# facebookresearch/theseus

Measured on NVIDIA H100. Metric: LM iterations/sec on batched SE3 pose-graph (2500 poses, global batch 2048 over N GPUs, LM + block-sparse Cholesky, fp64), higher is better.
Workload: dtype f64

## Files before the change

theseus_b200/_lib.py:

```python
import ctypes as C
import os

_HERE = os.path.dirname(os.path.abspath(__file__))
_LIB_PATH = os.environ.get("THB200_LIB") or os.path.join(_HERE, "lib", "libthb200.so")
_lib = None

c_i32, c_i64, c_f64, c_f32, c_vp = C.c_int32, C.c_int64, C.c_double, C.c_float, C.c_void_p


class CostGroup(C.Structure):
    _fields_ = [("kind", c_i32), ("weight_kind", c_i32), ("K", c_i32), ("dim", c_i32),
                ("x0", c_vp), ("x1", c_vp), ("aux", c_vp), ("w", c_vp), ("bstride", c_vp),
                ("a_off", c_vp), ("a_stride", c_vp), ("bp", c_vp), ("row0", c_vp),
                ("aux2", c_vp), ("aux3", c_vp), ("aux4", c_vp), ("bstride2", c_vp),
                ("robust_kind", c_i32), ("reserved0", c_i32), ("log_radius", c_vp), ("bstride_lr", c_vp),
                ("x2", c_vp), ("x3", c_vp), ("bstride3", c_vp), ("grid_rows", c_i32), ("grid_cols", c_i32)]


class VarTable(C.Structure):
    _fields_ = [("N", c_i32), ("x", c_vp), ("out", c_vp), ("kind", c_vp), ("col", c_vp), ("dof", c_vp)]


class GramPlan(C.Structure):
    _fields_ = [("num_entries", c_i64), ("ent_blk", c_vp), ("ent_p", c_vp), ("ent_q", c_vp),
                ("blk_out", c_vp), ("blk_ld", c_vp), ("blk_mirror", c_vp), ("blk_cptr", c_vp),
                ("c_off", c_vp), ("c_stride", c_vp), ("c_rows", c_vp), ("c_bpa", c_vp), ("c_bpb", c_vp),
                ("n", c_i64), ("col_cptr", c_vp), ("cc_off", c_vp), ("cc_stride", c_vp), ("cc_rows", c_vp),
                ("cc_row0", c_vp), ("num_blocks", c_i64), ("blk_rows", c_vp), ("blk_cols", c_vp),
                ("num_segments", c_i64), ("segments", c_vp), ("blk_order", c_vp)]


def make_gram_plan(arrs, dev):
    return GramPlan(
        num_entries=int(arrs["ent_blk"].shape[0]), ent_blk=dev["ent_blk"].data_ptr(), ent_p=dev["ent_p"].data_ptr(),
        ent_q=dev["ent_q"].data_ptr(), blk_out=dev["blk_out"].data_ptr(), blk_ld=dev["blk_ld"].data_ptr(),
        blk_mirror=dev["blk_mirror"].data_ptr(), blk_cptr=dev["blk_cptr"].data_ptr(), c_off=dev["c_off"].data_ptr(),
        c_stride=dev["c_stride"].data_ptr(), c_rows=dev["c_rows"].data_ptr(), c_bpa=dev["c_bpa"].data_ptr(),
        c_bpb=dev["c_bpb"].data_ptr(), n=int(arrs["n"]), col_cptr=dev["col_cptr"].data_ptr(),
        cc_off=dev["cc_off"].data_ptr(), cc_stride=dev["cc_stride"].data_ptr(), cc_rows=dev["cc_rows"].data_ptr(),
        cc_row0=dev["cc_row0"].data_ptr(), num_blocks=int(arrs["blk_out"].shape[0]), blk_rows=dev["blk_rows"].data_ptr(),
        blk_cols=dev["blk_cols"].data_ptr(), num_segments=int(arrs["segments"].shape[0]), segments=arrs["segments"].ctypes.data,
        blk_order=dev["blk_order"].data_ptr())


class SparsePlanStruct(C.Structure):
    _fields_ = [("N", c_i32), ("num_levels", c_i32), ("max_dim", c_i32), ("reserved", c_i32),
                ("n", c_i64), ("data_size", c_i64), ("winv_size", c_i64)] + [(k, c_vp) for k in (
                    "dims", "col_start", "pstart", "winv_off", "diag_off", "up_a", "up_b", "up_k",
                    "u_ptr", "u_tgt", "u_r", "u_c", "u_ld", "u_p0", "u_p1",
                    "f_ptr", "f_off", "f_dim", "f_w", "f_col",
                    "t_ptr", "t_off", "t_r", "t_dim", "t_w",
                    "s_ptr", "s_col", "fr_ptr", "fr_off", "fr_k", "bc_ptr", "bc_off", "bc_i")]


class SparseLanePlanStruct(C.Structure):
    _fields_ = [("N", c_i64), ("n", c_i64), ("data_size", c_i64), ("diag_size", c_i64), ("num_launches", c_i64)] + [(k, c_vp) for k in (
        "launches", "dims", "col_start", "pstart", "dl_off", "diag_off", "up_a", "up_b", "up_k", "u_tgt", "u_p0", "u_p1",
        "t_off", "t_diag", "t_dl", "t_pstart", "s_col", "fr_ptr", "fr_off", "fr_p", "fr_d", "bc_ptr", "bc_off", "bc_p", "bc_d")]


_PG, _PV, _PP = C.POINTER(CostGroup), C.POINTER(VarTable), C.POINTER(GramPlan)
_PS = C.POINTER(SparsePlanStruct)
_PL = C.POINTER(SparseLanePlanStruct)


class SparseLaneRootStruct(C.Structure):
    _fields_ = [("num_blocks", c_i64), ("num_cols", c_i64), ("nt", c_i64), ("root_start", c_i64), ("num_segments", c_i64)] + [(k, c_vp) for k in (
        "segments", "rb_off", "rb_row", "rb_col", "rb_di", "rb_dj", "rf_p0", "rf_p1", "root_cols", "root_dims")]


class SparseLaneTilesStruct(C.Structure):
    _fields_ = [("num_tiles", c_i64), ("num_steps", c_i64), ("tile_tgt", c_vp), ("step_ptr", c_vp), ("step_src", c_vp)]


class SparseLanePiecesStruct(C.Structure):
    _fields_ = [("num_pieces", c_i64), ("num_launches", c_i64)] + [(k, c_vp) for k in (
        "launches", "first", "width", "fr_ext_end", "bc_int_end", "order")]


class FrontPlanStruct(C.Structure):
    _fields_ = [("S", c_i64), ("n", c_i64), ("data_size", c_i64), ("arena_size", c_i64), ("varena_size", c_i64)] + [(k, c_vp) for k in (
        "f_w", "f_b", "f_first", "f_class", "f_wpad", "f_np", "f_cb_ld", "f_depth", "f_panel_off", "f_cb_off", "f_fr_off", "f_u_off",
        "child_ptr", "child_list", "rel_ptr", "f_rel", "rows_ptr", "f_rows", "sched", "perm", "c_jw", "c_sp_ptr", "c_sp", "c_inv_ptr", "c_inv", "fd", "pc", "pmap")]


_PF = C.POINTER(FrontPlanStruct)
_PR = C.POINTER(SparseLaneRootStruct)
_PPIECES = C.POINTER(SparseLanePiecesStruct)
_PT = C.POINTER(SparseLaneTilesStruct)
SIGNATURES = {
    "thb_version": (c_i32, []),
    "thb_compiled_arch": (c_i32, []),
    "thb_launch_count": (c_i64, []),
    "thb_linearize_group_f64": (c_i32, [_PG, c_i64, c_vp, c_i64, c_vp, c_i64, c_vp]),
    "thb_linearize_group_f32": (c_i32, [_PG, c_i64, c_vp, c_i64, c_vp, c_i64, c_vp]),
    "thb_error_num_chunks": (c_i32, [c_i32]),
    "thb_error_group_f64": (c_i32, [_PG, c_i64, c_vp, c_vp]),
    "thb_error_group_f32": (c_i32, [_PG, c_i64, c_vp, c_vp]),
    "thb_error_reduce_f64": (c_i32, [c_vp, c_i32, c_i64, c_vp, c_vp]),
    "thb_error_reduce_f32": (c_i32, [c_vp, c_i32, c_i64, c_vp, c_vp]),
    "thb_retract_f64": (c_i32, [_PV, c_i64, c_vp, c_i64, c_f64, c_vp, c_vp]),
    "thb_retract_f32": (c_i32, [_PV, c_i64, c_vp, c_i64, c_f32, c_vp, c_vp]),
    "thb_commit_f64": (c_i32, [_PV, c_i64, c_vp, c_vp]),
    "thb_commit_f32": (c_i32, [_PV, c_i64, c_vp, c_vp]),
    "thb_gram_f64": (c_i32, [_PP, c_i64, c_vp, c_i64, c_vp, c_i64, c_vp, c_i64, c_vp, c_vp, c_vp]),
    "thb_gram_f32": (c_i32, [_PP, c_i64, c_vp, c_i64, c_vp, c_i64, c_vp, c_i64, c_vp, c_vp, c_vp]),
    "thb_fill_zero": (c_i32, [c_vp, c_i64, c_vp]),
    "thb_potrf_workspace_bytes": (c_i64, [c_i64, c_i64]),
    "thb_potrf_f64": (c_i32, [c_vp, c_vp, c_vp, c_vp, c_i64, c_i64, c_vp, c_i64, c_vp]),
    "thb_potrs_f64": (c_i32, [c_vp, c_vp, c_i64, c_i64, c_vp, c_i64, c_vp]),
    "thb_potrf_potrs_f64": (c_i32, [c_vp, c_vp, c_vp, c_vp, c_vp, c_vp, c_i64, c_i64, c_vp, c_i64, c_vp]),
    "thb_sparse_damp_f64": (c_i32, [_PS, c_vp, c_vp, c_vp, c_i64, c_vp]),
    "thb_sparse_factor_f64": (c_i32, [_PS, c_vp, c_vp, c_vp, c_i64, c_vp]),
    "thb_sparse_solve_f64": (c_i32, [_PS, c_vp, c_vp, c_vp, c_vp, c_vp, c_i64, c_vp]),
    "thb_symbolic_create": (c_i32, [c_vp, c_i64, c_vp, c_vp, c_i32, c_vp]),
    "thb_symbolic_destroy": (None, [c_vp]),
    "thb_symbolic_array_count": (c_i64, [c_vp, C.c_char_p]),
    "thb_symbolic_array_elem_bytes": (c_i32, [c_vp, C.c_char_p]),
    "thb_symbolic_array_copy": (c_i32, [c_vp, C.c_char_p, c_vp, c_i64]),
    "thb_symbolic_stat": (C.c_double, [c_vp, C.c_char_p]),
    "thb_sparse_lane_padded_batch": (c_i64, [c_i64]),
    "thb_sparse_lane_gram_f64": (c_i32, [_PP, c_i64, c_vp, c_i64, c_vp, c_vp]),
    "thb_sparse_lane_damp_f64": (c_i32, [_PL, c_vp, c_vp, c_vp, c_i64, c_vp]),
    "thb_sparse_lane_factor_f64": (c_i32, [_PL, c_vp, c_vp, c_vp, c_i64, c_vp]),
    "thb_sparse_lane_factor_tiled_f64": (c_i32, [_PL, _PT, c_vp, c_vp, c_vp, c_i64, c_vp]),
    "thb_sparse_lane_solve_f64": (c_i32, [_PL, c_vp, c_vp, c_vp, c_vp, c_vp, c_i64, c_vp]),
    "thb_sparse_lane_forward_f64": (c_i32, [_PL, c_vp, c_vp, c_vp, c_vp, c_i64, c_vp]),
    "thb_sparse_lane_backward_f64": (c_i32, [_PL, c_vp, c_vp, c_vp, c_vp, c_i64, c_vp]),
    "thb_sparse_lane_piece_forward_f64": (c_i32, [_PL, _PPIECES, c_vp, c_vp, c_vp, c_vp, c_i64, c_vp]),
    "thb_sparse_lane_piece_backward_f64": (c_i32, [_PL, _PPIECES, c_vp, c_vp, c_vp, c_vp, c_i64, c_vp]),
    "thb_sparse_lane_root_gather_f64": (c_i32, [_PR, c_vp, c_vp, c_i64, c_vp]),
    "thb_sparse_lane_root_rhs_f64": (c_i32, [_PL, _PR, c_vp, c_vp, c_vp, c_vp, c_i64, c_vp]),
    "thb_sparse_lane_root_scatter_f64": (c_i32, [_PL, _PR, c_vp, c_vp, c_vp, c_i64, c_vp]),
    "thb_gram_dense_f64": (c_i32, [c_vp, c_vp, c_i64, c_i64, c_i64, c_vp]),
    "thb_front_small_smem_bytes": (c_i64, [c_i32, c_i32, c_i32]),
    "thb_front_factor_f64": (c_i32, [_PF, c_vp, c_i64, c_vp, c_vp, c_i64, c_vp, c_vp, c_vp, c_vp, c_i64, c_vp, c_i64, c_vp]),
    "thb_front_solve_f64": (c_i32, [_PF, c_vp, c_i64, c_vp, c_vp, c_vp, c_vp, c_vp, c_i64, c_vp]),
    "thb_front_factor_forward_f64": (c_i32, [_PF, c_vp, c_i64, c_vp, c_vp, c_i64, c_vp, c_vp, c_vp, c_vp, c_i64, c_vp, c_vp, c_vp, c_vp,
                                             c_i64, c_vp]),
    "thb_front_forward_f64": (c_i32, [_PF, c_vp, c_i64, c_vp, c_vp, c_vp, c_vp, c_i64, c_vp]),
    "thb_front_backward_f64": (c_i32, [_PF, c_vp, c_i64, c_vp, c_vp, c_vp, c_i64, c_vp]),
    "thb_potrf_partial_workspace_bytes": (c_i64, [c_i64, c_i64]),
    "thb_potrf_partial_inplace_f64": (c_i32, [c_vp, c_i64, c_i64, c_i32, c_i32, c_i32, c_i32, c_vp, c_i64, c_vp, c_i64, c_vp]),
    "thb_solve_backward_f64": (c_i32, [c_i64, c_i64, c_i64, c_vp, c_vp, c_vp, c_vp, c_vp, c_vp, c_vp, c_i32, c_vp, c_vp, c_vp]),
    "thb_lm_control_f64": (c_i32, [c_vp, c_vp, c_vp, c_i64, c_i64, c_f64, c_vp, c_vp, c_vp, c_i32, c_f64, c_f64, c_f64,
                                   c_vp, c_vp, c_vp, c_vp]),
    "thb_lm_control_f32": (c_i32, [c_vp, c_vp, c_vp, c_i64, c_i64, c_f32, c_vp, c_vp, c_vp, c_i32, c_f32, c_f32, c_f32,
                                   c_vp, c_vp, c_vp, c_vp]),
    "thb_mat_vec_f64": (c_i32, [c_i64, c_i64, c_i64, c_vp, c_vp, c_vp, c_vp, c_vp, c_vp]),
    "thb_tmat_vec_f64": (c_i32, [c_i64, c_i64, c_i64, c_vp, c_vp, c_vp, c_vp, c_vp, c_vp]),
}
for _sfx, _ in (("f64", c_f64), ("f32", c_f32)):
    SIGNATURES[f"thb_se3_exp_{_sfx}"] = (c_i32, [c_vp, c_vp, c_i64, c_vp])
    SIGNATURES[f"thb_se3_log_{_sfx}"] = (c_i32, [c_vp, c_vp, c_vp, c_i64, c_vp])
    SIGNATURES[f"thb_se3_adjoint_{_sfx}"] = (c_i32, [c_vp, c_vp, c_i64, c_vp])
    SIGNATURES[f"thb_se3_inverse_{_sfx}"] = (c_i32, [c_vp, c_vp, c_i64, c_vp])
    SIGNATURES[f"thb_se3_compose_{_sfx}"] = (c_i32, [c_vp, c_vp, c_vp, c_i64, c_vp])
    SIGNATURES[f"thb_se3_jexp_{_sfx}"] = (c_i32, [c_vp, c_vp, c_vp, c_i64, c_vp])
    SIGNATURES[f"thb_so3_jexp_{_sfx}"] = (c_i32, [c_vp, c_vp, c_vp, c_i64, c_vp])
    for _g in ("so3", "se2"):
        SIGNATURES[f"thb_{_g}_exp_{_sfx}"] = (c_i32, [c_vp, c_vp, c_i64, c_vp])
        SIGNATURES[f"thb_{_g}_log_{_sfx}"] = (c_i32, [c_vp, c_vp, c_vp, c_i64, c_vp])
        SIGNATURES[f"thb_{_g}_adjoint_{_sfx}"] = (c_i32, [c_vp, c_vp, c_i64, c_vp])
        SIGNATURES[f"thb_{_g}_inverse_{_sfx}"] = (c_i32, [c_vp, c_vp, c_i64, c_vp])
        SIGNATURES[f"thb_{_g}_compose_{_sfx}"] = (c_i32, [c_vp, c_vp, c_vp, c_i64, c_vp])


def lib_path():
    return _LIB_PATH


def load():
    global _lib
    if _lib is not None:
        return _lib
    if not os.path.exists(_LIB_PATH):
        raise RuntimeError(
            f"libthb200.so not found at {_LIB_PATH}: build it with `python -m theseus_b200.build` "
            "(theseus_b200 has no CPU or PyTorch fallback for its compute path)")
    import torch
    lib = C.CDLL(_LIB_PATH, mode=C.RTLD_GLOBAL)
    for name, (res, args) in SIGNATURES.items():
        fn = getattr(lib, name)
        fn.restype = res
        fn.argtypes = args
    _lib = lib
    return lib


replayed_launches = 0


def total_launches() -> int:
    return int(load().thb_launch_count()) + replayed_launches


def check(rc, what):
    if rc != 0:
        kind = "invalid argument" if rc < 0 else "CUDA error"
        raise RuntimeError(f"libthb200: {what} failed with {kind} code {rc}")


def stream_ptr():
    import torch
    return C.c_void_p(torch.cuda.current_stream().cuda_stream)


def ptr(t):
    return None if t is None else C.c_void_p(t.data_ptr())
```

theseus_b200/csrc/thb_front.cu:

```cuda
#include <stdlib.h>

#include "thb_common.cuh"

namespace thb {

#ifdef THB_SIMT_EMU
#define THB_PDL_TRIGGER() do { } while (0)
#define THB_PDL_WAIT() do { } while (0)
#define FRONT_LAUNCH(K, grid, block, smem, cs, arg) K<<<grid, block, smem, cs>>>(arg)
#else
#define THB_PDL_TRIGGER() asm volatile("griddepcontrol.launch_dependents;" ::: "memory")
#define THB_PDL_WAIT() asm volatile("griddepcontrol.wait;" ::: "memory")
#define FRONT_LAUNCH(K, grid, block, smem, cs, arg) thb::front_launch_pdl(K, grid, block, smem, cs, arg)
static inline bool front_pdl_enabled() {
  static const bool on = [] { const char* e = getenv("THB_FRONT_PDL"); return e != nullptr && e[0] == '1'; }();
  return on;
}
template <typename A>
static inline void front_launch_pdl(void (*kernel)(A), dim3 grid, dim3 block, size_t smem, cudaStream_t cs, const A& arg) {
  cudaLaunchConfig_t cfg = {};
  cfg.gridDim = grid; cfg.blockDim = block; cfg.dynamicSmemBytes = smem; cfg.stream = cs;
  cudaLaunchAttribute at[1];
  at[0].id = cudaLaunchAttributeProgrammaticStreamSerialization;
  at[0].val.programmaticStreamSerializationAllowed = 1;
  cfg.attrs = at; cfg.numAttrs = front_pdl_enabled() ? 1 : 0;
  cudaLaunchKernelEx(&cfg, kernel, arg);
}
#endif

#ifdef THB_SIMT_EMU
__device__ inline void front_mma884(double& c0, double& c1, double a, double b) {
  const int lane = threadIdx.x & 31, lr = lane >> 2, lc = lane & 3;
  for (int k = 0; k < 4; k++) {
    const double av = __shfl_sync(0xffffffffu, a, lr * 4 + k);
    const double b0 = __shfl_sync(0xffffffffu, b, (2 * lc) * 4 + k);
    const double b1 = __shfl_sync(0xffffffffu, b, (2 * lc + 1) * 4 + k);
    c0 += av * b0;
    c1 += av * b1;
  }
}
#else
__device__ __forceinline__ void front_mma884(double& c0, double& c1, double a, double b) {
  asm volatile("mma.sync.aligned.m8n8k4.row.col.f64.f64.f64.f64 {%0,%1}, {%2}, {%3}, {%0,%1};\n" : "+d"(c0), "+d"(c1) : "d"(a), "d"(b));
}
#endif

__host__ __device__ __forceinline__ int front_pad_ld(int x) { return ((x + 11) / 16) * 16 + 4; }

struct FrontArgs {
  thb_front_plan p;
  int s0;
  int64_t B;
  double* factor;
  const double* alpha;
  const double* beta;
  double* arena_cur;
  const double* arena_child;
  int32_t* info;
  int prefetch;
  const double* ata;
  int64_t ata_stride;
  const double* rhs;
  double* work;
  double* v_cur;
  const double* v_child;
};

__device__ __forceinline__ double front_panel_in(const FrontArgs& a, const double* Lg, int64_t poff, int64_t item, int64_t e) {
  if (a.ata == nullptr) return Lg[e];
  const int32_t m = a.p.pmap[poff + e];
  return m >= 0 ? a.ata[item * a.ata_stride + m] : 0.0;
}

constexpr int FRONT_WD_LD = 20;
#ifndef FRONT_PL
#define FRONT_PL 4
#endif
constexpr int FRONT_MAX_CHILDREN = 8;

__host__ __device__ __forceinline__ int64_t front_smem_doubles(int w, int b, int nchildren) {
  const int b16 = (b + 15) & ~15, w8 = (w + 7) & ~7;
  return (int64_t)(w8 + b16 + 8) * front_pad_ld(w8) + 8 * FRONT_WD_LD + 3 * FRONT_MAX_CHILDREN
         + ((int64_t)nchildren * (w + b) + 1) / 2 + 2;
}

__device__ __forceinline__ int front_leaf8(double* __restrict__ T, int ld, double* __restrict__ Wd, int lane) {
  const int ln = lane < 8 ? lane : 0;
  double row[8];
#pragma unroll
  for (int q = 0; q < 8; q++) row[q] = T[ln * ld + q];
  int fail = 0;
  double invd = 0.0;
#pragma unroll
  for (int c = 0; c < 8; c++) {
    const double d = __shfl_sync(0xffffffffu, row[c], c);
    if (!(d > 0.0) && fail == 0) fail = c + 1;
    double inv = rsqrt(d);
    inv = inv * (1.5 - 0.5 * d * inv * inv);
    const double sq = d * inv;
    if (lane == c) invd = inv;
    const double lrc = (lane == c) ? sq : row[c] * inv;
    row[c] = lrc;
#pragma unroll
    for (int q = c + 1; q < 8; q++) {
      const double lqc = __shfl_sync(0xffffffffu, lrc, q);
      row[q] -= lrc * lqc;
    }
  }
  if (lane < 8) {
#pragma unroll
    for (int q = 0; q < 8; q++)
      if (q <= lane) T[lane * ld + q] = row[q];
  }
  double x[8];
#pragma unroll
  for (int rr = 0; rr < 8; rr++) {
    double sacc = (lane == rr) ? 1.0 : 0.0;
#pragma unroll
    for (int k = 0; k < rr; k++) {
      const double lrk = __shfl_sync(0xffffffffu, row[k], rr);
      sacc -= lrk * x[k];
    }
    x[rr] = sacc * __shfl_sync(0xffffffffu, invd, rr);
  }
  if (lane < 8) {
#pragma unroll
    for (int rr = 0; rr < 8; rr++) Wd[rr * FRONT_WD_LD + lane] = (rr >= lane) ? x[rr] : 0.0;
  }
  return fail;
}

__device__ __forceinline__ void front_diag_block(double* PN, int ldp, int jb, double* Wd, int lane, int w, int first, int32_t* info) {
  const int lr = lane >> 2, lc = lane & 3;
  double c0 = 0.0, c1 = 0.0;
  const double* Arow = PN + (8 * jb + lr) * ldp + lc;
  for (int k = 0; k < 8 * jb; k += 4) {
    const double av = Arow[k];
    front_mma884(c0, c1, av, av);
  }
  double* d = PN + (8 * jb + lr) * ldp + 8 * jb + 2 * lc;
  d[0] -= c0;
  d[1] -= c1;
  __syncwarp();
  const int fail = front_leaf8(PN + (8 * jb) * ldp + 8 * jb, ldp, Wd, lane);
  if (lane == 0 && fail != 0 && 8 * jb + fail <= w) atomicCAS(info, 0, first + 8 * jb + fail);
}

template <bool TWO>
__device__ __forceinline__ void front_tile_column(double* PN, int ldp, int jb, int rt0, const double* Wd, int lane) {
  const int lr = lane >> 2, lc = lane & 3;
  double x00 = 0.0, x01 = 0.0, x10 = 0.0, x11 = 0.0;
  const double* A0 = PN + (8 * rt0 + lr) * ldp + lc;
  const double* Bj = PN + (8 * jb + lr) * ldp + lc;
  for (int k = 0; k < 8 * jb; k += 4) {
    const double bf = Bj[k];
    front_mma884(x00, x01, A0[k], bf);
    if (TWO) front_mma884(x10, x11, A0[8 * ldp + k], bf);
  }
  double* X0 = PN + (8 * rt0 + lr) * ldp + 8 * jb + 2 * lc;
  X0[0] -= x00; X0[1] -= x01;
  if (TWO) { X0[8 * ldp] -= x10; X0[8 * ldp + 1] -= x11; }
  __syncwarp();
  x00 = x01 = x10 = x11 = 0.0;
#pragma unroll
  for (int k = 0; k < 8; k += 4) {
    const double bf = Wd[lr * FRONT_WD_LD + k + lc];
    front_mma884(x00, x01, A0[8 * jb + k], bf);
    if (TWO) front_mma884(x10, x11, A0[8 * ldp + 8 * jb + k], bf);
  }
  __syncwarp();
  X0[0] = x00; X0[1] = x01;
  if (TWO) { X0[8 * ldp] = x10; X0[8 * ldp + 1] = x11; }
}

struct FrontChild {
  const double* src;
  int ldg, lo, hi, uoff;
};

__device__ __forceinline__ double front_warp_trsv_lower(const double* T, int ld, double ui, int cw, int lane) {
  const double rd = lane < cw ? 1.0 / T[lane * ld + lane] : 0.0;
  for (int k = 0; k < cw; k++) {
    const double yk = __shfl_sync(0xffffffffu, ui * rd, k);
    if (lane == k) ui = yk;
    else if (lane > k && lane < cw) ui -= T[lane * ld + k] * yk;
  }
  return ui;
}

struct FrontRowsGlobal {
  static constexpr bool kInPanel = false;
  const double* L;
  int w;
  double* T;
  __device__ __forceinline__ const double* row(int i) const { return L + (int64_t)i * w; }
  __device__ __forceinline__ const double* diag(int k0, int cw, int tid, int nthreads, int* ld) const {
    for (int e = tid; e < cw * cw; e += nthreads) {
      const int i = e / cw, j = e - i * cw;
      T[i * 33 + j] = L[(int64_t)(k0 + i) * w + k0 + j];
    }
    *ld = 33;
    return T;
  }
};
struct FrontRowsPanel {
  static constexpr bool kInPanel = true;
  const double* PN;
  int ldp, w, shift;
  __device__ __forceinline__ const double* row(int i) const { return PN + (i < w ? i : i + shift) * ldp; }
  __device__ __forceinline__ const double* diag(int k0, int, int, int, int* ld) const {
    *ld = ldp;
    return PN + k0 * ldp + k0;
  }
};

template <int THREADS, typename Rows>
__device__ __forceinline__ void front_forward_elim(const Rows& R, double* u, int us, int w, int r, int tid, int lane) {
  for (int k0 = 0; k0 < w; k0 += 32) {
    const int cw = min(32, w - k0);
    int ld;
    const double* T = R.diag(k0, cw, tid, THREADS, &ld);
    __syncthreads();
    if (tid < 32) {
      const double ui = front_warp_trsv_lower(T, ld, lane < cw ? u[(k0 + lane) * us] : 0.0, cw, lane);
      if (lane < cw) u[(k0 + lane) * us] = ui;
    }
    __syncthreads();
    for (int i = k0 + cw + tid; i < r; i += THREADS) {
      const double* row = R.row(i) + k0;
      double s = 0.0;
      if constexpr (Rows::kInPanel) {
#pragma unroll 2
        for (int k = 0; k < cw; k++) s += row[k] * u[(k0 + k) * us];
      } else {
        for (int k = 0; k < cw; k++) s += row[k] * u[(k0 + k) * us];
      }
      u[i * us] -= s;
    }
    __syncthreads();
  }
}

template <int THREADS>
__global__ void __launch_bounds__(THREADS, 1024 / THREADS) front_small_kernel(FrontArgs a) {
  extern __shared__ double sm[];
  const thb_front_plan& p = a.p;
  const int tid = threadIdx.x, lane = tid & 31, warp = tid >> 5;
  constexpr int NW = THREADS / 32;
  const int lr = lane >> 2, lc = lane & 3;
  const int64_t item = blockIdx.x;
  THB_PDL_TRIGGER();
  const int64_t* FD = p.fd + (int64_t)(a.s0 + blockIdx.y) * 8;
  const int t = (int)FD[0];
  const int w = (int)FD[1], b = (int)FD[2], r = w + b;
  const int f_first = (int)FD[3];
  const int64_t f_panel_off = FD[4], f_cb_off = FD[5];
  const int f_cb_ld = (int)FD[6];
  const int c_begin = (int)(FD[7] & 0xffffffffLL);
  const int nch = min((int)(FD[7] >> 32), FRONT_MAX_CHILDREN);
  const int b16 = (b + 15) & ~15, w8 = (w + 7) & ~7;
  const int ldp = front_pad_ld(w8);
  const int prow = w8 + b16 + 8;
  double* PN = sm;
  double* Wd = PN + prow * ldp;
  FrontChild* ch = reinterpret_cast<FrontChild*>(Wd + 8 * FRONT_WD_LD);
  int32_t* INV = reinterpret_cast<int32_t*>(Wd + 8 * FRONT_WD_LD + 3 * FRONT_MAX_CHILDREN);
  for (int q = 0; q < nch; q++) {
    const int64_t* PC = p.pc + (int64_t)(c_begin + q) * 6;
    const double* csrc = a.arena_child + item * p.arena_size + PC[0];
    const int cld = (int)(PC[1] & 0xffffffffLL), cbc = (int)(PC[1] >> 32);
    if (tid == 0) {
      ch[q].src = csrc;
      ch[q].ldg = cld;
      ch[q].lo = (int)PC[2];
      ch[q].hi = (int)PC[3];
      ch[q].uoff = (int)PC[5];
    }
    const int32_t* inv = p.c_inv + PC[4];
    for (int l = tid; l < r; l += THREADS) INV[q * r + l] = inv[l];
    (void)cbc;
  }
  for (int e = tid; e < prow * ldp; e += THREADS) sm[e] = 0.0;
  THB_PDL_WAIT();
#ifndef THB_SIMT_EMU
  if (a.rhs != nullptr) {
    for (int i = tid; i < w; i += THREADS) asm volatile("prefetch.global.L2 [%0];\n" ::"l"(a.rhs + item * p.n + p.perm[f_first + i]));
    for (int q = 0; q < nch; q++) {
      const int64_t* PC = p.pc + (int64_t)(c_begin + q) * 6;
      const double* cu = a.v_child + item * p.varena_size + PC[5];
      for (int off = tid * 16; off < (int)(PC[1] >> 32); off += THREADS * 16) asm volatile("prefetch.global.L2 [%0];\n" ::"l"(cu + off));
    }
  }
  for (int q = 0; a.prefetch != 0 && q < nch; q++) {
    const int64_t* PC = p.pc + (int64_t)(c_begin + q) * 6;
    const double* csrc = a.arena_child + item * p.arena_size + PC[0];
    const int cld = (int)(PC[1] & 0xffffffffLL), cbc = (int)(PC[1] >> 32);
    for (int off = tid * 16; off < cbc * cld; off += THREADS * 16) {
      const int i = off / cld, j = off - i * cld;
      if (j <= i) asm volatile("prefetch.global.L2 [%0];\n" ::"l"(csrc + off));
    }
  }
#endif
  __syncthreads();
  if (tid < w8 - w) PN[(w + tid) * ldp + w + tid] = 1.0;
  double* Lg = a.factor + item * p.data_size + f_panel_off;
  {
    const double al = a.alpha != nullptr ? a.alpha[item] : 0.0;
    const double be = a.beta != nullptr ? a.beta[item] : 0.0;
    const int total = r * w;
    for (int e0 = tid; e0 < total; e0 += FRONT_PL * THREADS) {
      int ii[FRONT_PL], jj[FRONT_PL];
      double v[FRONT_PL];
#pragma unroll
      for (int u = 0; u < FRONT_PL; u++) {
        const int e = e0 + u * THREADS;
        ii[u] = e / w;
        jj[u] = e - ii[u] * w;
        if (e >= total || jj[u] > ii[u]) ii[u] = -1;
        v[u] = ii[u] >= 0 ? front_panel_in(a, Lg, f_panel_off, item, e) : 0.0;
      }
#pragma unroll
      for (int u = 0; u < FRONT_PL; u++)
        if (ii[u] >= 0 && ii[u] == jj[u]) v[u] = v[u] + (al * v[u] + be);
      for (int q = 0; q < nch; q++) {
        const double* src = ch[q].src;
        const int ldg = ch[q].ldg, lo = ch[q].lo, hi = ch[q].hi;
        const int32_t* inv = INV + q * r;
#pragma unroll
        for (int u = 0; u < FRONT_PL; u++) {
          if (ii[u] >= lo && jj[u] <= hi) {
            const int ci = inv[ii[u]], cj = inv[jj[u]];
            if (ci >= 0 && cj >= 0) v[u] += src[(int64_t)ci * ldg + cj];
          }
        }
      }
#pragma unroll
      for (int u = 0; u < FRONT_PL; u++)
        if (ii[u] >= 0) PN[(ii[u] < w ? ii[u] : ii[u] + (w8 - w)) * ldp + jj[u]] = v[u];
    }
  }
  double* U = PN + w8;
  if (a.rhs != nullptr) {
    for (int i = tid; i < r; i += THREADS) {
      double v = i < w ? a.rhs[item * p.n + p.perm[f_first + i]] : 0.0;
      for (int q = 0; q < nch; q++) {
        if (i >= ch[q].lo && i <= ch[q].hi) {
          const int k = INV[q * r + i];
          if (k >= 0) v += a.v_child[item * p.varena_size + ch[q].uoff + k];
        }
      }
      U[i * ldp] = v;
    }
  }
  __syncthreads();
  const int nbk = w8 / 8, nrt = (w8 + b16) / 8;
  for (int jb = 0; jb < nbk; jb++) {
    if (warp == 0) front_diag_block(PN, ldp, jb, Wd, lane, w, f_first, a.info + item);
    __syncthreads();
    const int npair = (nrt - jb) / 2;
    for (int q = warp; q < npair; q += NW) front_tile_column<true>(PN, ldp, jb, jb + 1 + 2 * q, Wd, lane);
    __syncthreads();
  }
  {
    int i = tid / w, j = tid - i * w;
    const int di = THREADS / w, dj = THREADS - di * w;
    for (int e = tid; e < r * w; e += THREADS) {
      Lg[e] = (j > i) ? 0.0 : PN[(i < w ? i : i + (w8 - w)) * ldp + j];
      i += di; j += dj;
      if (j >= w) { j -= w; i++; }
    }
  }
  if (a.rhs != nullptr) {
    front_forward_elim<THREADS>(FrontRowsPanel{PN, ldp, w, w8 - w}, U, ldp, w, r, tid, lane);
    for (int i = tid; i < w; i += THREADS) a.work[item * p.n + f_first + i] = U[i * ldp];
    double* ub = a.v_cur + item * p.varena_size + p.f_u_off[t];
    for (int i = tid; i < b; i += THREADS) ub[i] = U[(w + i) * ldp];
  }
  if (b == 0) return;
  double* dst = a.arena_cur + item * p.arena_size + f_cb_off;
  const int ldg_out = f_cb_ld;
  const double* P = PN + w8 * ldp;
  const int nmt = b16 / 16, ntl = nmt * (nmt + 1) / 2;
  for (int q = warp; q < ntl; q += NW) {
    int R = (int)((sqrtf(8.0f * (float)q + 1.0f) - 1.0f) * 0.5f);
    while ((R + 1) * (R + 2) / 2 <= q) R++;
    while (R * (R + 1) / 2 > q) R--;
    const int ct = q - R * (R + 1) / 2;
    double gch[2][2][2] = {{{0.0, 0.0}, {0.0, 0.0}}, {{0.0, 0.0}, {0.0, 0.0}}};
    const int li0 = w + 16 * R + lr, lj0 = w + 16 * ct + 2 * lc;
    for (int qc = 0; qc < nch; qc++) {
      if (w + 16 * R + 15 >= ch[qc].lo && w + 16 * ct <= ch[qc].hi) {
        const int32_t* inv = INV + qc * r;
        const double* src = ch[qc].src;
        const int ldg = ch[qc].ldg;
        int ci[2], cj[2][2];
#pragma unroll
        for (int mi = 0; mi < 2; mi++) ci[mi] = (li0 + 8 * mi < r) ? inv[li0 + 8 * mi] : -1;
#pragma unroll
        for (int ni = 0; ni < 2; ni++)
#pragma unroll
          for (int u = 0; u < 2; u++) cj[ni][u] = (lj0 + 8 * ni + u < r) ? inv[lj0 + 8 * ni + u] : -1;
#pragma unroll
        for (int mi = 0; mi < 2; mi++)
#pragma unroll
          for (int ni = 0; ni < 2; ni++)
#pragma unroll
            for (int u = 0; u < 2; u++)
              if (ci[mi] >= 0 && cj[ni][u] >= 0 && cj[ni][u] <= ci[mi]) gch[mi][ni][u] += src[(int64_t)ci[mi] * ldg + cj[ni][u]];
      }
    }
    double acc[2][2][2] = {{{0.0, 0.0}, {0.0, 0.0}}, {{0.0, 0.0}, {0.0, 0.0}}};
    const double* Pa = P + (16 * R + lr) * ldp + lc;
    const double* Pb = P + (16 * ct + lr) * ldp + lc;
    for (int k4 = 0; k4 < w8; k4 += 4) {
      const double a0 = Pa[k4], a1 = Pa[8 * ldp + k4];
      const double b0 = Pb[k4], b1 = Pb[8 * ldp + k4];
      front_mma884(acc[0][0][0], acc[0][0][1], a0, b0);
      front_mma884(acc[0][1][0], acc[0][1][1], a0, b1);
      front_mma884(acc[1][0][0], acc[1][0][1], a1, b0);
      front_mma884(acc[1][1][0], acc[1][1][1], a1, b1);
    }
#pragma unroll
    for (int mi = 0; mi < 2; mi++)
#pragma unroll
      for (int ni = 0; ni < 2; ni++) {
        acc[mi][ni][0] = gch[mi][ni][0] - acc[mi][ni][0];
        acc[mi][ni][1] = gch[mi][ni][1] - acc[mi][ni][1];
      }
#pragma unroll
    for (int mi = 0; mi < 2; mi++) {
      const int i = 16 * R + 8 * mi + lr;
      if (i < b) {
        double* drow = dst + (int64_t)i * ldg_out;
#pragma unroll
        for (int ni = 0; ni < 2; ni++)
#pragma unroll
          for (int u = 0; u < 2; u++) {
            const int jj = 16 * ct + 8 * ni + 2 * lc + u;
            if (jj <= i) drow[jj] = acc[mi][ni][u];
          }
      }
    }
  }
}

constexpr int ASM_ROWS = 16, ASM_THREADS = 256;

__device__ __forceinline__ int front_map_big(int l, int w, int wpad) { return l < w ? l : wpad + (l - w); }

__global__ void __launch_bounds__(ASM_THREADS) front_assemble_kernel(FrontArgs a, int t) {
  extern __shared__ double sm[];
  const thb_front_plan& p = a.p;
  const int tid = threadIdx.x;
  const int64_t item = blockIdx.x;
  const int w = p.f_w[t], b = p.f_b[t], r = w + b, wpad = p.f_wpad[t], np = p.f_np[t];
  const int R0 = blockIdx.y * ASM_ROWS;
  const int nc = min(np, 128 * (R0 / 128 + 1));
  const int c_first = p.child_ptr[t], n_children = p.child_ptr[t + 1] - c_first;
  if (n_children <= FRONT_MAX_CHILDREN) {
    const double* Lgg = a.factor + item * p.data_size + p.f_panel_off[t];
    const double alg = a.alpha != nullptr ? a.alpha[item] : 0.0;
    const double beg = a.beta != nullptr ? a.beta[item] : 0.0;
    double* Fg = a.arena_cur + item * p.arena_size + p.f_fr_off[t] + (int64_t)R0 * np;
    __shared__ const double* s_src[FRONT_MAX_CHILDREN];
    __shared__ const int32_t* s_inv[FRONT_MAX_CHILDREN];
    __shared__ int s_ld[FRONT_MAX_CHILDREN];
    if (tid < n_children) {
      const int c = p.child_list[c_first + tid];
      s_src[tid] = a.arena_child + item * p.arena_size + p.f_cb_off[c];
      s_inv[tid] = p.c_inv + p.c_inv_ptr[c];
      s_ld[tid] = p.f_cb_ld[c];
    }
    __syncthreads();
    const int64_t poff = p.f_panel_off[t];
    const int total = ASM_ROWS * nc;
    for (int e0 = tid; e0 < total; e0 += 4 * ASM_THREADS) {
      int li[4], lj[4];
      double v[4];
#pragma unroll
      for (int u = 0; u < 4; u++) {
        const int e = e0 + u * ASM_THREADS;
        const int rr = e / nc, fc = e - rr * nc;
        const int fr = R0 + rr;
        li[u] = fr < w ? fr : ((fr >= wpad && fr - wpad + w < r) ? fr - wpad + w : -1);
        lj[u] = fc < w ? fc : ((fc >= wpad && fc - wpad + w < r) ? fc - wpad + w : -1);
        v[u] = 0.0;
        if (e >= total) {
          li[u] = lj[u] = -2;
        } else if (li[u] < 0 || lj[u] < 0) {
          v[u] = (fr == fc) ? 1.0 : 0.0;
          li[u] = -1;
        } else if (lj[u] > li[u]) {
          li[u] = -1;
        } else if (lj[u] < w) {
          v[u] = front_panel_in(a, Lgg, poff, item, (int64_t)li[u] * w + lj[u]);
        }
      }
#pragma unroll
      for (int u = 0; u < 4; u++)
        if (li[u] >= 0 && li[u] == lj[u] && lj[u] < w) v[u] = v[u] + (alg * v[u] + beg);
      for (int q = 0; q < n_children; q++) {
        const double* src = s_src[q];
        const int32_t* inv = s_inv[q];
        const int ldg = s_ld[q];
        int ci[4], cj[4];
#pragma unroll
        for (int u = 0; u < 4; u++) {
          ci[u] = li[u] >= 0 ? inv[li[u]] : -1;
          cj[u] = li[u] >= 0 ? inv[lj[u]] : -1;
        }
#pragma unroll
        for (int u = 0; u < 4; u++)
          if (ci[u] >= 0 && cj[u] >= 0) v[u] += src[(int64_t)ci[u] * ldg + cj[u]];
      }
#pragma unroll
      for (int u = 0; u < 4; u++) {
        const int e = e0 + u * ASM_THREADS;
        if (e < total) Fg[e + (int64_t)(e / nc) * (np - nc)] = v[u];
      }
    }
    return;
  }
  double* buf = sm;
  for (int e = tid; e < ASM_ROWS * nc; e += ASM_THREADS) buf[e] = 0.0;
  __syncthreads();
  const double* Lg = a.factor + item * p.data_size + p.f_panel_off[t];
  const double al = a.alpha != nullptr ? a.alpha[item] : 0.0;
  const double be = a.beta != nullptr ? a.beta[item] : 0.0;
  const int wlim = min(wpad, nc);
  for (int e = tid; e < ASM_ROWS * wlim; e += ASM_THREADS) {
    const int rr = e / wlim, j = e - rr * wlim;
    const int fr = R0 + rr;
    int i = -1;
    if (fr < w) i = fr;
    else if (fr >= wpad && fr - wpad + w < r) i = fr - wpad + w;
    if (i >= 0) {
      if (j < w && !(i < w && j > i)) {
        double v = front_panel_in(a, Lg, p.f_panel_off[t], item, (int64_t)i * w + j);
        if (i == j) v = v + (al * v + be);
        buf[rr * nc + j] = v;
      }
    } else if (j == fr) {
      buf[rr * nc + j] = 1.0;
    }
  }
  for (int rr = tid; rr < ASM_ROWS; rr += ASM_THREADS) {
    const int fr = R0 + rr;
    if (fr >= wpad + b) buf[rr * nc + fr] = 1.0;
  }
  __syncthreads();
  for (int ci = p.child_ptr[t]; ci < p.child_ptr[t + 1]; ci++) {
    const int c = p.child_list[ci];
    const int bc = p.f_b[c], ldg = p.f_cb_ld[c];
    const int32_t* rel = p.f_rel + p.rel_ptr[c];
    int lo = 0, hi = bc;
    while (lo < hi) { const int mid = (lo + hi) >> 1; if (front_map_big(rel[mid], w, wpad) < R0) lo = mid + 1; else hi = mid; }
    const int i0 = lo;
    hi = bc;
    while (lo < hi) { const int mid = (lo + hi) >> 1; if (front_map_big(rel[mid], w, wpad) < R0 + ASM_ROWS) lo = mid + 1; else hi = mid; }
    const int i1 = lo;
    if (i1 > i0) {
      const double* src = a.arena_child + item * p.arena_size + p.f_cb_off[c];
      for (int i = i0 + (tid >> 5); i < i1; i += ASM_THREADS / 32) {
        const int fr = front_map_big(rel[i], w, wpad) - R0;
        const double* srow = src + (int64_t)i * ldg;
        for (int j = tid & 31; j <= i; j += 32) buf[fr * nc + front_map_big(rel[j], w, wpad)] += srow[j];
      }
      __syncthreads();
    }
  }
  double* F = a.arena_cur + item * p.arena_size + p.f_fr_off[t] + (int64_t)R0 * np;
  for (int e = tid; e < ASM_ROWS * nc; e += ASM_THREADS) {
    const int rr = e / nc, c = e - rr * nc;
    F[(int64_t)rr * np + c] = buf[e];
  }
}

__global__ void __launch_bounds__(256) front_extract_kernel(FrontArgs a, int t) {
  const thb_front_plan& p = a.p;
  const int64_t item = blockIdx.x;
  const int w = p.f_w[t], b = p.f_b[t], r = w + b, wpad = p.f_wpad[t], np = p.f_np[t];
  const double* F = a.arena_cur + item * p.arena_size + p.f_fr_off[t];
  double* Lg = a.factor + item * p.data_size + p.f_panel_off[t];
  for (int e = blockIdx.y * blockDim.x + threadIdx.x; e < r * w; e += gridDim.y * blockDim.x) {
    const int i = e / w, j = e - i * w;
    const int fr = i < w ? i : wpad + (i - w);
    Lg[e] = (i < w && j > i) ? 0.0 : F[(int64_t)fr * np + j];
  }
}

struct FrontSolveArgs {
  thb_front_plan p;
  int s0;
  int64_t B;
  const double* factor;
  const double* rhs;
  double* x;
  double* work;
  double* v_cur;
  const double* v_child;
  int stage_doubles;
};

__device__ __forceinline__ double front_warp_trsv_upper(const double* T, double ti, int cw, int lane) {
  const double rd = lane < cw ? 1.0 / T[lane * 33 + lane] : 0.0;
  for (int k = cw - 1; k >= 0; k--) {
    const double xk = __shfl_sync(0xffffffffu, ti * rd, k);
    if (lane == k) ti = xk;
    else if (lane < k) ti -= T[k * 33 + lane] * xk;
  }
  return ti;
}

template <int THREADS>
__global__ void __launch_bounds__(THREADS) front_forward_kernel(FrontSolveArgs a) {
  extern __shared__ double sm[];
  const thb_front_plan& p = a.p;
  const int tid = threadIdx.x, lane = tid & 31;
  const int64_t item = blockIdx.x;
  THB_PDL_TRIGGER();
  const int64_t* FD = p.fd + (int64_t)(a.s0 + blockIdx.y) * 8;
  const int t = (int)FD[0];
  const int w = (int)FD[1], b = (int)FD[2], r = w + b, first = (int)FD[3];
  THB_PDL_WAIT();
  double* u = sm;
  double* T = sm + ((r + 1) & ~1);
  const double* Lg = a.factor + item * p.data_size + FD[4];
  if (r * w <= a.stage_doubles) {
    double* Ls = T + 32 * 33 + 1 + (THREADS & ~1) + 2;
    for (int e = tid; e < r * w; e += THREADS) Ls[e] = Lg[e];
    Lg = Ls;
  }
  {
    const int c0 = (int)(FD[7] & 0xffffffffLL), nchild = (int)(FD[7] >> 32);
    for (int i = tid; i < r; i += THREADS) {
      double v = i < w ? a.rhs[item * p.n + p.perm[first + i]] : 0.0;
      for (int q = 0; q < nchild; q++) {
        const int64_t* PC = p.pc + (int64_t)(c0 + q) * 6;
        if (i >= (int)PC[2] && i <= (int)PC[3]) {
          const int k = p.c_inv[PC[4] + i];
          if (k >= 0) v += a.v_child[item * p.varena_size + PC[5] + k];
        }
      }
      u[i] = v;
    }
  }
  __syncthreads();
  front_forward_elim<THREADS>(FrontRowsGlobal{Lg, w, T}, u, 1, w, r, tid, lane);
  for (int i = tid; i < w; i += THREADS) a.work[item * p.n + first + i] = u[i];
  if (b > 0) {
    double* ub = a.v_cur + item * p.varena_size + p.f_u_off[t];
    for (int i = tid; i < b; i += THREADS) ub[i] = u[w + i];
  }
}

template <int THREADS>
__global__ void __launch_bounds__(THREADS) front_backward_kernel(FrontSolveArgs a) {
  extern __shared__ double sm[];
  const thb_front_plan& p = a.p;
  const int tid = threadIdx.x, lane = tid & 31, warp = tid >> 5;
  const int64_t item = blockIdx.x;
  THB_PDL_TRIGGER();
  const int64_t* FD = p.fd + (int64_t)(a.s0 + blockIdx.y) * 8;
  const int t = (int)FD[0];
  const int w = (int)FD[1], b = (int)FD[2], r = w + b, first = (int)FD[3];
  THB_PDL_WAIT();
  double* xf = sm;
  double* T = sm + ((r + 1) & ~1);
  double* part = T + 32 * 33 + 1;
  const double* Lg = a.factor + item * p.data_size + FD[4];
  if (r * w <= a.stage_doubles) {
    double* Ls = T + 32 * 33 + 1 + (THREADS & ~1) + 2;
    for (int e = tid; e < r * w; e += THREADS) Ls[e] = Lg[e];
    Lg = Ls;
  }
  double* wk = a.work + item * p.n;
  const int32_t* rows = p.f_rows + p.rows_ptr[t];
  for (int i = tid; i < r; i += THREADS) xf[i] = i < w ? wk[first + i] : wk[rows[i - w]];
  __syncthreads();
  const int nchunk = (w + 31) / 32;
  for (int ch = nchunk - 1; ch >= 0; ch--) {
    const int k0 = ch * 32, cw = min(32, w - k0);
    const int RG = THREADS / cw;
    const int kk = tid % cw, rg = tid / cw;
    for (int e = tid; e < cw * cw; e += THREADS) {
      const int i = e / cw, j = e - i * cw;
      T[i * 33 + j] = Lg[(int64_t)(k0 + i) * w + k0 + j];
    }
    double acc = 0.0;
    if (rg < RG) {
      const double* col = Lg + k0 + kk;
      int i = k0 + cw + rg;
      for (; i + 3 * RG < r; i += 4 * RG) {
        const double l0 = col[(int64_t)i * w], l1 = col[(int64_t)(i + RG) * w], l2 = col[(int64_t)(i + 2 * RG) * w],
                     l3 = col[(int64_t)(i + 3 * RG) * w];
        acc += l0 * xf[i];
        acc += l1 * xf[i + RG];
        acc += l2 * xf[i + 2 * RG];
        acc += l3 * xf[i + 3 * RG];
      }
      for (; i < r; i += RG) acc += col[(int64_t)i * w] * xf[i];
    }
    part[tid] = acc;
    __syncthreads();
    if (warp == 0) {
      double tk = 0.0;
      if (lane < cw) {
        tk = xf[k0 + lane];
        for (int g = 0; g < RG; g++) tk -= part[g * cw + lane];
      }
      tk = front_warp_trsv_upper(T, tk, cw, lane);
      if (lane < cw) xf[k0 + lane] = tk;
    }
    __syncthreads();
  }
  for (int i = tid; i < w; i += THREADS) {
    const double v = xf[i];
    wk[first + i] = v;
    a.x[item * p.n + p.perm[first + i]] = v;
  }
}

static inline int front_threads_of_class(int cls) { return cls == 0 ? 64 : (cls == 1 ? 128 : 256); }

template <typename K>
static inline int front_set_smem(K kernel, size_t bytes, size_t* cache) {
  if (bytes > *cache) {
    cudaError_t e = cudaFuncSetAttribute(kernel, cudaFuncAttributeMaxDynamicSharedMemorySize, (int)bytes);
    if (e != cudaSuccess) return (int)e;
    *cache = bytes;
  }
  return 0;
}

static int front_solve_launch(const thb_front_plan* p, const int64_t* L, int pass, const double* factor, const double* rhs, double* x,
                              double* work, double* varena, int64_t B, cudaStream_t cs) {
  static size_t fw_set[3] = {0, 0, 0}, bw_set[3] = {0, 0, 0};
  static const int64_t stage_cap = [] { const char* e = getenv("THB_SOLVE_STAGE"); return e != nullptr ? (int64_t)atoll(e) : (int64_t)0; }();
  const int depth = (int)L[0], cls = (int)L[1], begin = (int)L[2], count = (int)L[3];
  FrontSolveArgs a;
  a.p = *p; a.s0 = begin; a.B = B; a.factor = factor; a.rhs = rhs; a.x = x; a.work = work;
  a.v_cur = varena != nullptr ? varena + (int64_t)(depth & 1) * B * p->varena_size : nullptr;
  a.v_child = varena != nullptr ? varena + (int64_t)((depth + 1) & 1) * B * p->varena_size : nullptr;
  const int kc = cls > 2 ? 2 : cls;
  const int threads = front_threads_of_class(kc);
  const int64_t r_max = L[5];
  const int64_t stage = (cls < 3 && L[6] > 0) ? (L[6] < stage_cap ? L[6] : stage_cap) : 0;
  a.stage_doubles = (int)stage;
  const size_t smem = (size_t)(((r_max + 1) & ~1LL) + 32 * 33 + 1 + threads + 2 + stage + 2) * 8;
  const dim3 grid((unsigned)B, (unsigned)count);
  if (pass == 0) {
    if (kc == 0) { int rc = front_set_smem(front_forward_kernel<64>, smem, &fw_set[0]); if (rc) return rc;
                   FRONT_LAUNCH(front_forward_kernel<64>, grid, 64, smem, cs, a); }
    else if (kc == 1) { int rc = front_set_smem(front_forward_kernel<128>, smem, &fw_set[1]); if (rc) return rc;
                        FRONT_LAUNCH(front_forward_kernel<128>, grid, 128, smem, cs, a); }
    else { int rc = front_set_smem(front_forward_kernel<256>, smem, &fw_set[2]); if (rc) return rc;
           FRONT_LAUNCH(front_forward_kernel<256>, grid, 256, smem, cs, a); }
  } else {
    if (kc == 0) { int rc = front_set_smem(front_backward_kernel<64>, smem, &bw_set[0]); if (rc) return rc;
                   FRONT_LAUNCH(front_backward_kernel<64>, grid, 64, smem, cs, a); }
    else if (kc == 1) { int rc = front_set_smem(front_backward_kernel<128>, smem, &bw_set[1]); if (rc) return rc;
                        FRONT_LAUNCH(front_backward_kernel<128>, grid, 128, smem, cs, a); }
    else { int rc = front_set_smem(front_backward_kernel<256>, smem, &bw_set[2]); if (rc) return rc;
           FRONT_LAUNCH(front_backward_kernel<256>, grid, 256, smem, cs, a); }
  }
  THB_CHECK_LAUNCH();
  return THB_OK;
}

static int front_factor(const thb_front_plan* p, const int64_t* launches, int64_t num_launches, double* factor, const double* ata,
                        int64_t ata_stride, const double* alpha, const double* beta, double* arena, void* dense_ws, int64_t dense_ws_bytes,
                        int32_t* info, const double* rhs, double* work, double* varena, int64_t B, thb_stream_t stream) {
  if (p == nullptr || launches == nullptr || factor == nullptr || arena == nullptr || info == nullptr || B < 0) return THB_ERR_BAD_ARG;
  if (B == 0 || p->S == 0) return THB_OK;
  if (B > 65535LL * 32768LL) return THB_ERR_UNSUPPORTED;
  cudaStream_t cs = thb_cs(stream);
  THB_CUDA(cudaMemsetAsync(info, 0, (size_t)B * 4, cs));
  static size_t smem_set[5] = {0, 0, 0, 0, 0}, asm_set = 0;
  static const int thr_cls[2] = {[] { const char* e = getenv("THB_FRONT_T0"); const int v = e ? atoi(e) : 64; return (v == 128 || v == 256) ? v : 64; }(),
                                 [] { const char* e = getenv("THB_FRONT_T1"); const int v = e ? atoi(e) : 128; return v == 256 ? 256 : 128; }()};
  static int front_prefetch_flag = -1;
  if (front_prefetch_flag < 0) {
    const char* e = getenv("THB_FRONT_PREFETCH");
    front_prefetch_flag = (e != nullptr && e[0] == '1') ? 1 : 0;
  }
  static const int fuse_max = [] { const char* e = getenv("THB_FRONT_FUSE_MAX"); return e != nullptr ? atoi(e) : 1024; }();
  for (int64_t l = 0; l < num_launches; l++) {
    const int64_t* L = launches + l * THB_FRONT_LAUNCH_COLS;
    const int depth = (int)L[0], cls = (int)L[1], begin = (int)L[2], count = (int)L[3];
    FrontArgs a;
    a.p = *p; a.s0 = begin; a.B = B; a.factor = factor; a.alpha = alpha; a.beta = beta; a.info = info;
    a.ata = (ata != nullptr && p->pmap != nullptr) ? ata : nullptr; a.ata_stride = ata_stride;
    a.prefetch = front_prefetch_flag;
    a.arena_cur = arena + (int64_t)(depth & 1) * B * p->arena_size;
    a.arena_child = arena + (int64_t)((depth + 1) & 1) * B * p->arena_size;
    a.rhs = rhs; a.work = work;
    a.v_cur = rhs != nullptr ? varena + (int64_t)(depth & 1) * B * p->varena_size : nullptr;
    a.v_child = rhs != nullptr ? varena + (int64_t)((depth + 1) & 1) * B * p->varena_size : nullptr;
    if (cls < 3) {
      const size_t smem = (size_t)L[4];
#ifndef THB_SIMT_EMU
      if (smem > 227 * 1024) return THB_ERR_UNSUPPORTED;
#endif
      const dim3 grid((unsigned)B, (unsigned)count);
      if (count > 65535) return THB_ERR_UNSUPPORTED;
      const int threads = (cls == 0 && thr_cls[0] == 64) ? 64
                          : ((cls == 0 && thr_cls[0] == 128) || (cls == 1 && thr_cls[1] == 128)) ? 128
                          : (cls <= 1 || smem <= 56 * 1024) ? 256 : (smem <= 113 * 1024 ? 512 : 1024);
      const bool fused = rhs != nullptr && threads <= fuse_max;
      if (!fused) a.rhs = nullptr;
      if (threads == 64) {
        int rc = front_set_smem(front_small_kernel<64>, smem, &smem_set[0]); if (rc) return rc;
        FRONT_LAUNCH(front_small_kernel<64>, grid, 64, smem, cs, a);
      } else if (threads == 128) {
        int rc = front_set_smem(front_small_kernel<128>, smem, &smem_set[1]); if (rc) return rc;
        FRONT_LAUNCH(front_small_kernel<128>, grid, 128, smem, cs, a);
      } else if (threads == 256) {
        int rc = front_set_smem(front_small_kernel<256>, smem, &smem_set[2]); if (rc) return rc;
        FRONT_LAUNCH(front_small_kernel<256>, grid, 256, smem, cs, a);
      } else if (threads == 512) {
        int rc = front_set_smem(front_small_kernel<512>, smem, &smem_set[3]); if (rc) return rc;
        FRONT_LAUNCH(front_small_kernel<512>, grid, 512, smem, cs, a);
      } else {
        int rc = front_set_smem(front_small_kernel<1024>, smem, &smem_set[4]); if (rc) return rc;
        FRONT_LAUNCH(front_small_kernel<1024>, grid, 1024, smem, cs, a);
      }
      THB_CHECK_LAUNCH();
      if (rhs != nullptr && !fused) {
        const int rc = front_solve_launch(p, L, 0, factor, rhs, nullptr, work, varena, B, cs);
        if (rc != THB_OK) return rc;
      }
    } else {
      const int64_t np = L[5], nb_piv = L[6], fr_off = L[7], first = L[8];
      const int t = (int)L[9];
#ifdef THB_SIMT_EMU
      (void)np; (void)nb_piv; (void)fr_off; (void)first; (void)t; (void)dense_ws; (void)dense_ws_bytes; (void)asm_set;
      return THB_ERR_UNSUPPORTED;
#else
      if (dense_ws == nullptr || np % 128 != 0 || np > 8192) return THB_ERR_BAD_ARG;
      const size_t smem = (size_t)ASM_ROWS * np * 8;
      int rc = front_set_smem(front_assemble_kernel, smem, &asm_set); if (rc) return rc;
      front_assemble_kernel<<<dim3((unsigned)B, (unsigned)(np / ASM_ROWS)), ASM_THREADS, smem, cs>>>(a, t);
      THB_CHECK_LAUNCH();
      rc = thb_potrf_partial_inplace_f64(a.arena_cur + fr_off, p->arena_size, np, (int32_t)nb_piv, (int32_t)L[10], (int32_t)(nb_piv * 64 + L[11]),
                                         (int32_t)first, info, B, dense_ws, dense_ws_bytes, stream);
      if (rc != THB_OK) return rc;
      front_extract_kernel<<<dim3((unsigned)B, 8), 256, 0, cs>>>(a, t);
      THB_CHECK_LAUNCH();
      if (rhs != nullptr) {
        rc = front_solve_launch(p, L, 0, factor, rhs, nullptr, work, varena, B, cs);
        if (rc != THB_OK) return rc;
      }
#endif
    }
  }
  return THB_OK;
}

}

extern "C" {

int64_t thb_front_small_smem_bytes(int32_t w, int32_t b, int32_t nchildren) { return thb::front_smem_doubles(w, b, nchildren) * 8; }

int thb_front_factor_f64(const thb_front_plan* p, const int64_t* launches, int64_t num_launches, double* factor, const double* ata,
                         int64_t ata_stride, const double* alpha, const double* beta, double* arena, void* dense_ws, int64_t dense_ws_bytes,
                         int32_t* info, int64_t B, thb_stream_t stream) {
  return thb::front_factor(p, launches, num_launches, factor, ata, ata_stride, alpha, beta, arena, dense_ws, dense_ws_bytes, info, nullptr,
                           nullptr, nullptr, B, stream);
}

int thb_front_factor_forward_f64(const thb_front_plan* p, const int64_t* launches, int64_t num_launches, double* factor, const double* ata,
                                 int64_t ata_stride, const double* alpha, const double* beta, double* arena, void* dense_ws,
                                 int64_t dense_ws_bytes, int32_t* info, const double* rhs, double* work, double* varena, int64_t B,
                                 thb_stream_t stream) {
  if (rhs == nullptr || work == nullptr || varena == nullptr) return THB_ERR_BAD_ARG;
  return thb::front_factor(p, launches, num_launches, factor, ata, ata_stride, alpha, beta, arena, dense_ws, dense_ws_bytes, info, rhs, work,
                           varena, B, stream);
}

int thb_front_solve_f64(const thb_front_plan* p, const int64_t* launches, int64_t num_launches, const double* factor, const double* rhs,
                        double* x, double* work, double* varena, int64_t B, thb_stream_t stream) {
  if (p == nullptr || launches == nullptr || factor == nullptr || rhs == nullptr || x == nullptr || work == nullptr || varena == nullptr ||
      B < 0)
    return THB_ERR_BAD_ARG;
  if (B == 0 || p->S == 0) return THB_OK;
  const int rc = thb_front_forward_f64(p, launches, num_launches, factor, rhs, work, varena, B, stream);
  if (rc != THB_OK) return rc;
  return thb_front_backward_f64(p, launches, num_launches, factor, x, work, B, stream);
}

int thb_front_forward_f64(const thb_front_plan* p, const int64_t* launches, int64_t num_launches, const double* factor, const double* rhs,
                          double* work, double* varena, int64_t B, thb_stream_t stream) {
  if (p == nullptr || launches == nullptr || factor == nullptr || rhs == nullptr || work == nullptr || varena == nullptr || B < 0)
    return THB_ERR_BAD_ARG;
  if (B == 0 || p->S == 0) return THB_OK;
  cudaStream_t cs = thb_cs(stream);
  for (int64_t q = 0; q < num_launches; q++) {
    const int rc = thb::front_solve_launch(p, launches + q * THB_FRONT_LAUNCH_COLS, 0, factor, rhs, nullptr, work, varena, B, cs);
    if (rc != THB_OK) return rc;
  }
  return THB_OK;
}

int thb_front_backward_f64(const thb_front_plan* p, const int64_t* launches, int64_t num_launches, const double* factor, double* x,
                           double* work, int64_t B, thb_stream_t stream) {
  if (p == nullptr || launches == nullptr || factor == nullptr || x == nullptr || work == nullptr || B < 0) return THB_ERR_BAD_ARG;
  if (B == 0 || p->S == 0) return THB_OK;
  cudaStream_t cs = thb_cs(stream);
  for (int64_t q = num_launches - 1; q >= 0; q--) {
    const int rc = thb::front_solve_launch(p, launches + q * THB_FRONT_LAUNCH_COLS, 1, factor, nullptr, x, work, nullptr, B, cs);
    if (rc != THB_OK) return rc;
  }
  return THB_OK;
}

}
```

theseus_b200/extlib.py:

```python
import ctypes as C
from typing import Dict, Tuple

import numpy as np
import torch

from . import _lib
from .frontal import FrontPlan, build_front_plan


class SymbolicDecomposition:
    def __init__(self, param_size: torch.Tensor, sparse_struct_ptrs: torch.Tensor, sparse_struct_inds: torch.Tensor, dev: str = "cuda"):
        if str(dev) not in ("cuda",) and not str(dev).startswith("cuda"):
            raise RuntimeError("theseus_b200.extlib: only dev='cuda' exists (no CPU implementation of the factorisation in this package)")
        ps = np.asarray(param_size.cpu().numpy() if torch.is_tensor(param_size) else param_size, dtype=np.int64)
        ptrs = np.asarray(sparse_struct_ptrs.cpu().numpy() if torch.is_tensor(sparse_struct_ptrs) else sparse_struct_ptrs, dtype=np.int64)
        inds = np.asarray(sparse_struct_inds.cpu().numpy() if torch.is_tensor(sparse_struct_inds) else sparse_struct_inds, dtype=np.int64)
        N = int(ps.shape[0])
        if ptrs.shape[0] != N + 1:
            raise RuntimeError("sparse_struct_ptrs must have len(param_size) + 1 entries")
        nbr = [set([i]) for i in range(N)]
        for i in range(N):
            for j in inds[ptrs[i]:ptrs[i + 1]]:
                nbr[i].add(int(j)); nbr[int(j)].add(i)
        fp = np.zeros(N + 1, dtype=np.int64)
        fi = []
        for i in range(N):
            fi.extend(sorted(nbr[i])); fp[i + 1] = len(fi)
        self.param_size = ps
        self.plan: FrontPlan = build_front_plan(ps, fp, np.array(fi, dtype=np.int64))
        self.device = torch.device(dev if str(dev) != "cuda" else "cuda")
        self.param_start = np.concatenate([[0], np.cumsum(ps)[:-1]]).astype(np.int64)
        self.to_param = np.repeat(np.arange(N), ps)
        self._dev = None
        self._tables: Dict[Tuple, Tuple[torch.Tensor, ...]] = {}

    def create_numeric_decomposition(self, batch_size: int) -> "NumericDecomposition":
        return NumericDecomposition(self, int(batch_size))

    def _device_plan(self):
        if self._dev is None:
            P = self.plan
            dev = {k: torch.from_numpy(np.ascontiguousarray(v)).to(self.device) for k, v in P.arrays.items()}
            keys = ("f_w", "f_b", "f_first", "f_class", "f_wpad", "f_np", "f_cb_ld", "f_depth", "f_panel_off", "f_cb_off", "f_fr_off", "f_u_off",
                    "child_ptr", "child_list", "rel_ptr", "f_rel", "rows_ptr", "f_rows", "sched", "perm", "c_jw", "c_sp_ptr", "c_sp", "c_inv_ptr", "c_inv", "fd", "pc", "pmap")
            st = _lib.FrontPlanStruct(S=P.S, n=P.n, data_size=P.data_size, arena_size=P.arena_size, varena_size=P.varena_size,
                                      **{k: dev[k].data_ptr() for k in keys})
            launches = np.ascontiguousarray(P.launches, dtype=np.int64)
            big = launches[launches[:, 1] == 3]
            self._dev = dict(front=st, keep=dev, launches=launches, max_np=int(big[:, 5].max()) if len(big) else 0)
        return self._dev

    def _offset_of(self, r: np.ndarray, c: np.ndarray) -> np.ndarray:
        P = self.plan
        A = P.arrays
        pr, pc = self.to_param[r], self.to_param[c]
        posr, posc = P.pos[pr], P.pos[pc]
        swap = posr < posc
        r2, c2 = np.where(swap, c, r), np.where(swap, r, c)
        pr, pc = self.to_param[r2], self.to_param[c2]
        posr, posc = P.pos[pr], P.pos[pc]
        same = posr == posc
        sw2 = same & (r2 < c2)
        r2, c2 = np.where(sw2, c2, r2), np.where(sw2, r2, c2)
        gr = P.pstart[posr] + (r2 - self.param_start[pr])
        gc = P.pstart[posc] + (c2 - self.param_start[pc])
        s = P.front_of_pos[posc]
        first, w = A["f_first"][s].astype(np.int64), A["f_w"][s].astype(np.int64)
        lcol = gc - first
        out = np.empty(r.shape[0], dtype=np.int64)
        for k in range(r.shape[0]):
            if gr[k] < first[k] + w[k]:
                lrow = gr[k] - first[k]
                if lrow < lcol[k]:
                    lrow, lc = lcol[k], gr[k] - first[k]
                    out[k] = A["f_panel_off"][s[k]] + lrow * w[k] + lc
                    continue
            else:
                rows = P.border_rows[int(s[k])]
                j = int(np.searchsorted(rows, gr[k]))
                assert rows[j] == gr[k], "entry outside the symbolic structure"
                lrow = w[k] + j
            out[k] = A["f_panel_off"][s[k]] + lrow * w[k] + lcol[k]
        return out

    def _add_m_table(self, ptrs: np.ndarray, inds: np.ndarray):
        key = ("M", ptrs.tobytes(), inds.tobytes())
        if key not in self._tables:
            rows = np.repeat(np.arange(ptrs.shape[0] - 1), np.diff(ptrs))
            keep = np.nonzero(inds <= rows)[0]
            off = self._offset_of(rows[keep], inds[keep])
            self._tables[key] = (torch.from_numpy(keep).to(self.device), torch.from_numpy(off).to(self.device))
        return self._tables[key]

    def _add_mtm_table(self, ptrs: np.ndarray, inds: np.ndarray):
        key = ("MtM", ptrs.tobytes(), inds.tobytes())
        if key not in self._tables:
            jj, ii = [], []
            for q in range(ptrs.shape[0] - 1):
                a, b = int(ptrs[q]), int(ptrs[q + 1])
                for j in range(a, b):
                    for i in range(a, j + 1):
                        jj.append(j); ii.append(i)
            jj, ii = np.array(jj, dtype=np.int64), np.array(ii, dtype=np.int64)
            off = self._offset_of(inds[jj], inds[ii])
            order = np.argsort(off, kind="stable")
            self._tables[key] = tuple(torch.from_numpy(x[order]).to(self.device) for x in (jj, ii, off))
        return self._tables[key]

    def _diag_offsets(self):
        if "diag" not in self._tables:
            idx = np.arange(self.plan.n)
            self._tables["diag"] = (torch.from_numpy(self._offset_of(idx, idx)).to(self.device),)
        return self._tables["diag"][0]


class NumericDecomposition:
    def __init__(self, symbolic: SymbolicDecomposition, batch_size: int):
        self.sym, self.B = symbolic, batch_size
        P = symbolic.plan
        self.data = torch.zeros(batch_size, P.data_size, dtype=torch.float64, device=symbolic.device)
        self._bufs = None

    @staticmethod
    def _np(t):
        return np.ascontiguousarray(t.cpu().numpy() if torch.is_tensor(t) else t, dtype=np.int64)

    def add_M(self, val: torch.Tensor, ptrs, inds):
        keep, off = self.sym._add_m_table(self._np(ptrs), self._np(inds))
        self.data.index_add_(1, off, val.to(self.data.device, torch.float64)[:, keep])

    def add_MtM(self, val: torch.Tensor, ptrs, inds):
        jj, ii, off = self.sym._add_mtm_table(self._np(ptrs), self._np(inds))
        v = val.to(self.data.device, torch.float64)
        self.data.index_add_(1, off, v[:, jj] * v[:, ii])

    def damp(self, alpha: torch.Tensor, beta: torch.Tensor):
        d = self.sym._diag_offsets()
        diag = self.data[:, d]
        self.data[:, d] = diag * (1.0 + alpha.to(diag).view(-1, 1)) + beta.to(diag).view(-1, 1)

    def _buffers(self):
        if self._bufs is None:
            P, dev = self.sym.plan, self.sym._device_plan()
            lib = _lib.load()
            ws_bytes = int(lib.thb_potrf_partial_workspace_bytes(self.B, dev["max_np"])) if dev["max_np"] else 0
            kw = dict(dtype=torch.float64, device=self.data.device)
            self._bufs = dict(arena=torch.empty(2, self.B, P.arena_size, **kw), varena=torch.empty(2, self.B, P.varena_size, **kw),
                              work=torch.empty(self.B, P.n, **kw), ws=torch.empty(max(ws_bytes, 8), dtype=torch.uint8, device=self.data.device),
                              info=torch.empty(self.B, dtype=torch.int32, device=self.data.device))
        return self._bufs

    def factor(self):
        dev, bufs, lib = self.sym._device_plan(), self._buffers(), _lib.load()
        L = dev["launches"]
        _lib.check(lib.thb_front_factor_f64(C.byref(dev["front"]), L.ctypes.data, L.shape[0], _lib.ptr(self.data), None, 0, None, None, _lib.ptr(bufs["arena"]),
                                            _lib.ptr(bufs["ws"]) if dev["max_np"] else None, bufs["ws"].numel(), _lib.ptr(bufs["info"]), self.B,
                                            _lib.stream_ptr()), "front_factor")
        bad = bufs["info"].nonzero()
        if bad.numel() > 0:
            k = int(bad[0, 0])
            raise RuntimeError(f"block-sparse Cholesky: batch element {k}: matrix is not positive definite (pivot {int(bufs['info'][k])})")

    def solve(self, x: torch.Tensor):
        dev, bufs, lib = self.sym._device_plan(), self._buffers(), _lib.load()
        L = dev["launches"]
        rhs = x.detach().to(torch.float64).contiguous().clone()
        out = torch.empty_like(rhs)
        _lib.check(lib.thb_front_solve_f64(C.byref(dev["front"]), L.ctypes.data, L.shape[0], _lib.ptr(self.data), _lib.ptr(rhs), _lib.ptr(out),
                                           _lib.ptr(bufs["work"]), _lib.ptr(bufs["varena"]), self.B, _lib.stream_ptr()), "front_solve")
        x.copy_(out)
        return x
```

theseus_b200/frontal.py:

```python
from dataclasses import dataclass, field
from typing import Dict, List, Optional

import numpy as np

SMALL_CLASSES = (48, 96, 1 << 30)
BIG_TW, BIG_TM = 64, 128


def _bfs_levels(adj, start, mask, stamp, mark):
    mark[start] = True
    levels, seen = [[start]], [start]
    while True:
        nxt = []
        for u in levels[-1]:
            for v in adj[u]:
                if mask[v] == stamp and not mark[v]:
                    mark[v] = True
                    nxt.append(v)
                    seen.append(v)
        if not nxt:
            break
        levels.append(nxt)
    for v in seen:
        mark[v] = False
    return levels, seen


def nested_dissection_order(N: int, ptrs: np.ndarray, inds: np.ndarray, leaf: int = 8) -> np.ndarray:
    adj = [[int(x) for x in inds[ptrs[i]:ptrs[i + 1]] if int(x) != i] for i in range(N)]
    mask = np.zeros(N, dtype=np.int64)
    mark = np.zeros(N, dtype=bool)
    order: List[int] = []
    stamp = [0]
    work = [("nodes", list(range(N)))]
    while work:
        kind, nodes = work.pop()
        if kind == "emit":
            order.extend(nodes)
            continue
        if not nodes:
            continue
        stamp[0] += 1
        s = stamp[0]
        for v in nodes:
            mask[v] = s
        if len(nodes) <= leaf:
            order.extend(sorted(nodes, key=lambda v: (sum(1 for x in adj[v] if mask[x] == s), v)))
            for v in nodes:
                mask[v] = 0
            continue
        remaining = set(nodes)
        comps = []
        for v in nodes:
            if v in remaining:
                _, seen = _bfs_levels(adj, v, mask, s, mark)
                comps.append(seen)
                remaining.difference_update(seen)
        if len(comps) > 1:
            for c in reversed(comps):
                work.append(("nodes", c))
            continue
        levels, _ = _bfs_levels(adj, nodes[0], mask, s, mark)
        for _ in range(4):
            cand = min(levels[-1], key=lambda v: (sum(1 for x in adj[v] if mask[x] == s), v))
            l2, _ = _bfs_levels(adj, cand, mask, s, mark)
            if len(l2) > len(levels):
                levels = l2
            else:
                break
        if len(levels) < 3:
            order.extend(sorted(nodes))
            for v in nodes:
                mask[v] = 0
            continue
        tot = len(nodes)
        cum = np.cumsum([len(l) for l in levels])
        best, bi = None, None
        for i in range(1, len(levels) - 1):
            left, right = int(cum[i - 1]), tot - int(cum[i])
            bal = min(left, right) / max(left, right, 1)
            if bal < 0.4:
                continue
            score = (len(levels[i]), -bal)
            if best is None or score < best:
                best, bi = score, i
        if bi is None:
            bi = min(max(int(np.argmin(np.abs(cum - tot / 2))), 1), len(levels) - 2)
        right = [v for l in levels[bi + 1:] for v in l]
        left = [v for l in levels[:bi] for v in l]
        rs = set(right)
        sep = []
        for v in levels[bi]:
            if any((x in rs) for x in adj[v]):
                sep.append(v)
            else:
                left.append(v)
        for v in sep:
            mask[v] = 0
        work.append(("emit", sorted(sep)))
        work.append(("nodes", right))
        work.append(("nodes", left))
    assert len(order) == N
    return np.array(order, dtype=np.int64)


def _column_structures(N, ptrs, inds, order):
    pos = np.empty(N, dtype=np.int64)
    pos[order] = np.arange(N)
    parent = -np.ones(N, dtype=np.int64)
    struct: List[Optional[set]] = [None] * N
    children: List[List[int]] = [[] for _ in range(N)]
    for j in range(N):
        v = int(order[j])
        s = set(int(pos[x]) for x in inds[ptrs[v]:ptrs[v + 1]] if pos[x] > j)
        for c in children[j]:
            s.update(struct[c])
        s.discard(j)
        struct[j] = s
        if s:
            p = min(s)
            parent[j] = p
            children[p].append(j)
    return pos, parent, [np.array(sorted(s), dtype=np.int64) for s in struct]


def _flops_of(struct, dims):
    fl = 0.0
    for j, s in enumerate(struct):
        r = float(sum(dims[i] for i in s))
        d = float(dims[j])
        fl += d ** 3 / 3.0 + d * d * r + d * r * r
    return fl


STRIPE = 32
SMALL_SMEM_LIMIT = 220 * 1024
SMEM_BUCKETS = (27 * 1024, 36 * 1024, 55 * 1024, 74 * 1024, 112 * 1024)


def _pad_ld(x: int) -> int:
    return ((x + 11) // 16) * 16 + 4


def small_smem_bytes(w: int, b: int, nchildren: int = 0) -> int:
    b16, w8 = (b + 15) & ~15, (w + 7) & ~7
    return ((w8 + b16 + 8) * _pad_ld(w8) + 8 * 20 + 3 * SMALL_MAX_CHILDREN + 2 + (min(nchildren, SMALL_MAX_CHILDREN) * (w + b) + 1) // 2) * 8


SPLIT_MAX_W = int(__import__("os").environ.get("THB_FRONT_SPLIT_W", "96"))
SPLIT_ROOT_W = 256
SMALL_MAX_CHILDREN = 8
SMALL_MAX_W = 192


def _front_cost(w, b):
    return w ** 3 / 3.0 + w * w * b + w * b * b


@dataclass
class FrontPlan:
    N: int
    n: int
    param_size: np.ndarray
    order: np.ndarray
    pos: np.ndarray
    dims: np.ndarray
    pstart: np.ndarray
    col_start: np.ndarray
    perm: np.ndarray
    S: int
    arrays: Dict[str, np.ndarray]
    launches: np.ndarray
    data_size: int
    arena_size: int
    varena_size: int
    stats: Dict[str, float] = field(default_factory=dict)
    front_of_pos: np.ndarray = None
    border_rows: List[np.ndarray] = None

    def gram_compact_offsets(self, blocks_dims):
        f = self.gram_out_offsets()
        pmap = self.arrays["pmap"]
        pmap[:] = -1
        table, off = {}, 0
        for (a, b, di, dj) in blocks_dims:
            po, ld, _ = f(a, b)
            idx = po + np.arange(di)[:, None] * ld + np.arange(dj)[None, :]
            pmap[idx] = off + np.arange(di)[:, None] * dj + np.arange(dj)[None, :]
            table[(a, b)] = (off, dj, -1)
            off += di * dj
        return (lambda a, b: table[(int(a), int(b))]), off

    def gram_out_offsets(self):
        A = self.arrays
        first, w, poff = A["f_first"], A["f_w"], A["f_panel_off"]

        def f(a: int, b: int):
            pa, pb = int(self.pos[a]), int(self.pos[b])
            s = int(self.front_of_pos[pb])
            lcol = int(self.pstart[pb] - first[s])
            ga = int(self.pstart[pa])
            if ga < first[s] + w[s]:
                lrow = ga - int(first[s])
            else:
                k = int(np.searchsorted(self.border_rows[s], ga))
                assert self.border_rows[s][k] == ga
                lrow = int(w[s]) + k
            return int(poff[s]) + lrow * int(w[s]) + lcol, int(w[s]), -1
        return f


def build_front_plan(param_size, ptrs, inds, ordering: str = "auto", tau: float = 0.12, merge_flops: float = 4e4,
                     merge_max_r: int = SMALL_CLASSES[1], small_limit: Optional[int] = None, split_wide: bool = True) -> FrontPlan:
    param_size = np.asarray(param_size, dtype=np.int64)
    ptrs = np.asarray(ptrs, dtype=np.int64)
    inds = np.asarray(inds, dtype=np.int64)
    N = int(param_size.shape[0])
    from .sparse import minimum_degree_order
    cands = {}
    if ordering in ("auto", "nd"):
        cands["nd"] = nested_dissection_order(N, ptrs, inds)
    if ordering in ("auto", "mindeg"):
        cands["mindeg"] = minimum_degree_order(N, ptrs, inds, param_size)
    if ordering == "natural":
        cands["natural"] = np.arange(N, dtype=np.int64)
    if not cands:
        raise ValueError(ordering)
    best = None
    for name, o in cands.items():
        pos0, parent, struct = _column_structures(N, ptrs, inds, o)
        fl = _flops_of(struct, param_size[o])
        if best is None or fl < best[0]:
            best = (fl, name, o, pos0, parent, struct)
    col_flops, oname, order0, pos0, parent, struct = best
    dims0 = param_size[order0]

    nchild = np.zeros(N, dtype=np.int64)
    for j in range(N):
        if parent[j] >= 0:
            nchild[parent[j]] += 1
    firsts = [0]
    for j in range(1, N):
        if not (parent[j - 1] == j and len(struct[j - 1]) == len(struct[j]) + 1 and nchild[j] == 1):
            firsts.append(j)
    firsts.append(N)
    sn = [(firsts[i], firsts[i + 1]) for i in range(len(firsts) - 1)]
    S0 = len(sn)
    sn_of = np.empty(N, dtype=np.int64)
    for s, (a, b) in enumerate(sn):
        sn_of[a:b] = s
    cols = [list(range(a, b)) for a, b in sn]
    below = [struct[b - 1] for a, b in sn]
    wsz = [int(dims0[a:b].sum()) for a, b in sn]
    bsz = [int(dims0[struct[b - 1]].sum()) if len(struct[b - 1]) else 0 for a, b in sn]
    par = np.array([sn_of[parent[b - 1]] if parent[b - 1] >= 0 else -1 for a, b in sn], dtype=np.int64)
    kids: List[List[int]] = [[] for _ in range(S0)]
    for s in range(S0):
        if par[s] >= 0:
            kids[par[s]].append(s)
    alive = np.ones(S0, dtype=bool)
    base = [_front_cost(wsz[s], bsz[s]) for s in range(S0)]
    for p in range(S0):
        changed = True
        while changed and kids[p]:
            changed = False
            for c in sorted(kids[p], key=lambda c: (wsz[c] + bsz[c], c)):
                sep = base[c] + base[p]
                mer = _front_cost(wsz[c] + wsz[p], bsz[p])
                r_m = wsz[c] + wsz[p] + bsz[p]
                if mer <= (1.0 + tau) * sep or (mer <= sep + merge_flops and r_m <= merge_max_r):
                    cols[p] = cols[c] + cols[p]
                    wsz[p] += wsz[c]
                    base[p] = sep
                    alive[c] = False
                    kids[p].remove(c)
                    for g in kids[c]:
                        par[g] = p
                        kids[p].append(g)
                    kids[c] = []
                    changed = True
                    break
    fr_cols: List[List[int]] = []
    fr_below: List[np.ndarray] = []
    for sidx in (q for q in range(S0) if alive[q]):
        cs, bl = cols[sidx], np.asarray(below[sidx], dtype=np.int64)
        wtot, btot = int(dims0[cs].sum()), (int(dims0[bl].sum()) if len(bl) else 0)
        fits = wtot <= SMALL_MAX_W and small_smem_bytes(wtot, btot, 4) <= SMALL_SMEM_LIMIT
        if fits or not split_wide or (btot == 0 and wtot > SPLIT_ROOT_W):
            fr_cols.append(list(cs)); fr_below.append(bl)
            continue
        pieces, i0 = [], 0
        while i0 < len(cs):
            i1, wacc = i0, 0
            rest = int(dims0[cs[i0:]].sum())
            while i1 < len(cs):
                wn = wacc + int(dims0[cs[i1]])
                if i1 > i0 and (wn > SPLIT_MAX_W or small_smem_bytes(wn, rest - wn + btot, 4) > SMALL_SMEM_LIMIT):
                    break
                wacc, i1 = wn, i1 + 1
            pieces.append((i0, i1))
            i0 = i1
        if any(small_smem_bytes(int(dims0[cs[a:b_]].sum()), int(dims0[cs[b_:]].sum()) + btot, 4) > SMALL_SMEM_LIMIT for a, b_ in pieces):
            fr_cols.append(list(cs)); fr_below.append(bl)
            continue
        for a, b_ in pieces:
            fr_cols.append(list(cs[a:b_]))
            fr_below.append(np.concatenate([np.asarray(cs[b_:], dtype=np.int64), bl]))
    S = len(fr_cols)
    keep = list(range(S))
    cols, below = fr_cols, fr_below
    old_positions = np.array([j for s in keep for j in cols[s]], dtype=np.int64)
    assert sorted(old_positions.tolist()) == list(range(N))
    newpos_of_old = np.empty(N, dtype=np.int64)
    newpos_of_old[old_positions] = np.arange(N)
    order = order0[old_positions]
    pos = np.empty(N, dtype=np.int64)
    pos[order] = np.arange(N)
    dims = param_size[order]
    pstart = np.concatenate([[0], np.cumsum(dims)[:-1]]).astype(np.int64)
    n = int(dims.sum())
    orig_start = np.concatenate([[0], np.cumsum(param_size)[:-1]]).astype(np.int64)
    col_start = orig_start[order]
    perm = np.concatenate([np.arange(col_start[k], col_start[k] + dims[k]) for k in range(N)]).astype(np.int64) if N else np.zeros(0, np.int64)

    f_w = np.zeros(S, dtype=np.int32)
    f_b = np.zeros(S, dtype=np.int32)
    f_first = np.zeros(S, dtype=np.int32)
    f_parent = -np.ones(S, dtype=np.int32)
    front_of_pos = np.empty(N, dtype=np.int64)
    border_rows: List[np.ndarray] = []
    k0 = 0
    for t, s in enumerate(keep):
        nc = len(cols[s])
        front_of_pos[k0:k0 + nc] = t
        f_first[t] = pstart[k0]
        f_w[t] = int(dims[k0:k0 + nc].sum())
        bp = np.sort(newpos_of_old[below[s]]) if len(below[s]) else np.zeros(0, dtype=np.int64)
        assert len(bp) == 0 or bp[0] >= k0 + nc
        rows = np.concatenate([np.arange(pstart[q], pstart[q] + dims[q]) for q in bp]).astype(np.int64) if len(bp) else np.zeros(0, np.int64)
        border_rows.append(rows)
        f_b[t] = rows.shape[0]
        k0 += nc
    for t in range(S):
        if f_b[t] > 0:
            first_row_pos = int(np.searchsorted(pstart, border_rows[t][0], side="right") - 1)
            f_parent[t] = int(front_of_pos[first_row_pos])
            assert f_parent[t] > t
    f_r = f_w + f_b
    f_depth = np.zeros(S, dtype=np.int32)
    for t in range(S - 1, -1, -1):
        if f_parent[t] >= 0:
            f_depth[t] = f_depth[f_parent[t]] + 1
    max_depth = int(f_depth.max()) if S else 0
    children: List[List[int]] = [[] for _ in range(S)]
    for t in range(S):
        if f_parent[t] >= 0:
            children[f_parent[t]].append(t)
    f_class = np.zeros(S, dtype=np.int32)
    for t in range(S):
        r = int(f_r[t])
        too_big = (small_limit is not None and r > small_limit) or int(f_w[t]) > SMALL_MAX_W or \
            small_smem_bytes(int(f_w[t]), int(f_b[t]), len(children[t])) > SMALL_SMEM_LIMIT or len(children[t]) > SMALL_MAX_CHILDREN
        f_class[t] = 3 if too_big else min(int(np.searchsorted(np.array(SMALL_CLASSES), r)), 2)
    f_panel_off = np.zeros(S, dtype=np.int64)
    off = 0
    for t in range(S):
        f_panel_off[t] = off
        off += int(f_r[t]) * int(f_w[t])
        off += off & 1
    data_size = off
    f_wpad = np.zeros(S, dtype=np.int32)
    f_np = np.zeros(S, dtype=np.int32)
    f_cb_off = np.zeros(S, dtype=np.int64)
    f_cb_ld = np.zeros(S, dtype=np.int32)
    f_fr_off = np.zeros(S, dtype=np.int64)
    f_u_off = np.zeros(S, dtype=np.int64)
    arena = [0, 0]
    varena = [0, 0]
    for d in range(max_depth, -1, -1):
        a = 0
        v = 0
        for t in np.nonzero(f_depth == d)[0]:
            if f_class[t] == 3:
                wp = -(-int(f_w[t]) // BIG_TW) * BIG_TW
                npad = -(-(wp + int(f_b[t])) // BIG_TM) * BIG_TM
                f_wpad[t], f_np[t] = wp, npad
                f_fr_off[t] = a
                f_cb_off[t] = a + wp * npad + wp
                f_cb_ld[t] = npad
                a += npad * npad
            else:
                ld = int(f_b[t]) + (int(f_b[t]) & 1)
                f_cb_off[t] = a
                f_cb_ld[t] = ld
                a += int(f_b[t]) * ld
            f_u_off[t] = v
            v += int(f_b[t]) + (int(f_b[t]) & 1)
        arena[d & 1] = max(arena[d & 1], a)
        varena[d & 1] = max(varena[d & 1], v)
    arena_size = max(arena) + 2
    varena_size = max(varena) + 2
    child_ptr = np.zeros(S + 1, dtype=np.int32)
    child_list: List[int] = []
    rel_ptr = np.zeros(S + 1, dtype=np.int64)
    rel_list: List[np.ndarray] = []
    for t in range(S):
        child_list.extend(children[t])
        child_ptr[t + 1] = len(child_list)
    racc = 0
    for t in range(S):
        p = int(f_parent[t])
        if p >= 0:
            g = border_rows[t]
            inp = g < f_first[p] + f_w[p]
            loc = np.where(inp, g - f_first[p], f_w[p] + np.searchsorted(border_rows[p], g))
            if len(border_rows[p]):
                kk = np.clip(loc - f_w[p], 0, len(border_rows[p]) - 1)
                assert bool(np.all(inp | (border_rows[p][kk] == g)))
            else:
                assert bool(np.all(inp))
            assert bool(np.all(g >= f_first[p]))
            rel_list.append(loc.astype(np.int32))
            racc += len(loc)
        rel_ptr[t + 1] = racc
    f_rel = np.concatenate(rel_list).astype(np.int32) if rel_list else np.zeros(0, dtype=np.int32)
    c_jw = np.zeros(S, dtype=np.int32)
    c_sp_ptr = np.zeros(S + 1, dtype=np.int64)
    c_sp_list: List[np.ndarray] = []
    acc = 0
    for t in range(S):
        p = int(f_parent[t])
        if p >= 0:
            rel = f_rel[rel_ptr[t]:rel_ptr[t + 1]]
            c_jw[t] = int(np.searchsorted(rel, int(f_w[p])))
            ns = -(-int(f_b[p]) // STRIPE) + 1
            sp = np.searchsorted(rel, int(f_w[p]) + STRIPE * np.arange(ns)).astype(np.int32)
            c_sp_list.append(sp)
            acc += ns
        c_sp_ptr[t + 1] = acc
    c_sp = np.concatenate(c_sp_list).astype(np.int32) if c_sp_list else np.zeros(1, dtype=np.int32)
    c_inv_ptr = np.zeros(S + 1, dtype=np.int64)
    c_inv_list: List[np.ndarray] = []
    acc = 0
    for t in range(S):
        p = int(f_parent[t])
        if p >= 0:
            inv = -np.ones(int(f_r[p]), dtype=np.int32)
            rel = f_rel[rel_ptr[t]:rel_ptr[t + 1]]
            inv[rel] = np.arange(rel.shape[0], dtype=np.int32)
            c_inv_list.append(inv)
            acc += inv.shape[0]
        c_inv_ptr[t + 1] = acc
    c_inv = np.concatenate(c_inv_list).astype(np.int32) if c_inv_list else np.zeros(1, dtype=np.int32)
    rows_ptr = np.zeros(S + 1, dtype=np.int64)
    rows_ptr[1:] = np.cumsum(f_b)
    f_rows = np.concatenate(border_rows).astype(np.int32) if S else np.zeros(0, dtype=np.int32)
    def bucket(t):
        if f_class[t] == 3:
            return 0
        sm = small_smem_bytes(int(f_w[t]), int(f_b[t]), len(children[t]))
        return int(np.searchsorted(np.array(SMEM_BUCKETS), sm))
    f_bucket = np.array([bucket(t) for t in range(S)], dtype=np.int32)
    sched = np.array(sorted(range(S), key=lambda t: (-int(f_depth[t]), int(f_class[t]), int(f_bucket[t]), -int(f_r[t]), t)), dtype=np.int32)
    launches = []
    i = 0
    while i < S:
        t = int(sched[i])
        d, c, bk = int(f_depth[t]), int(f_class[t]), int(f_bucket[t])
        j = i + 1
        if c != 3:
            while j < S and int(f_depth[sched[j]]) == d and int(f_class[sched[j]]) == c and int(f_bucket[sched[j]]) == bk:
                j += 1
            smem = max(small_smem_bytes(int(f_w[q]), int(f_b[q]), len(children[q])) for q in sched[i:j])
            launches.append((d, c, i, j - i, smem, max(int(f_r[q]) for q in sched[i:j]), max(int(f_r[q]) * int(f_w[q]) for q in sched[i:j]),
                             0, 0, 0, 0, 0))
        else:
            launches.append((d, c, i, 1, 0, int(f_np[t]), int(f_wpad[t]) // BIG_TW, int(f_fr_off[t]), int(f_first[t]), t, int(f_w[t]), int(f_b[t])))
        i = j
    launches = np.array(launches, dtype=np.int64).reshape(-1, 12)
    fd = np.zeros((max(S, 1), 8), dtype=np.int64)
    pc = np.zeros((max(int(child_ptr[S]), 1), 6), dtype=np.int64)
    for q in range(S):
        t = int(sched[q])
        cb, ce = int(child_ptr[t]), int(child_ptr[t + 1])
        fd[q] = (t, int(f_w[t]), int(f_b[t]), int(f_first[t]), int(f_panel_off[t]), int(f_cb_off[t]), int(f_cb_ld[t]), cb | ((ce - cb) << 32))
    for t in range(S):
        for k, c in enumerate(children[t]):
            rel = f_rel[rel_ptr[c]:rel_ptr[c + 1]]
            pc[int(child_ptr[t]) + k] = (int(f_cb_off[c]), int(f_cb_ld[c]) | (int(f_b[c]) << 32), int(rel[0]), int(rel[-1]), int(c_inv_ptr[c]),
                                         int(f_u_off[c]))
    flops = float(sum(_front_cost(float(f_w[t]), float(f_b[t])) for t in range(S)))
    stats = dict(ordering=oname, column_flops=col_flops, flops=flops, nnz_L=float(sum(int(f_r[t]) * int(f_w[t]) for t in range(S))),
                 fronts=float(S), max_front=float(f_r.max()) if S else 0.0, depth=float(max_depth + 1), big_fronts=float((f_class == 3).sum()),
                 launches=float(len(launches)), cb_doubles=float(sum(int(b) * int(b) for b in f_b)), levels=float(max_depth + 1),
                 num_updates=0.0, num_chains=float(S), chain_levels=float(max_depth + 1))
    arrays = dict(f_w=f_w, f_b=f_b, f_first=f_first, f_parent=f_parent, f_depth=f_depth, f_class=f_class, f_panel_off=f_panel_off,
                  f_wpad=f_wpad, f_np=f_np, f_cb_off=f_cb_off, f_cb_ld=f_cb_ld, f_fr_off=f_fr_off, f_u_off=f_u_off,
                  child_ptr=child_ptr, child_list=np.array(child_list, dtype=np.int32), rel_ptr=rel_ptr, f_rel=f_rel,
                  rows_ptr=rows_ptr, f_rows=f_rows, sched=sched, perm=perm.astype(np.int32), c_jw=c_jw, c_sp_ptr=c_sp_ptr, c_sp=c_sp,
                  c_inv_ptr=c_inv_ptr, c_inv=c_inv, fd=fd.reshape(-1), pc=pc.reshape(-1),
                  pmap=-np.ones(max(int(data_size), 1), dtype=np.int32))
    return FrontPlan(N=N, n=n, param_size=param_size, order=order, pos=pos, dims=dims, pstart=pstart, col_start=col_start, perm=perm, S=S,
                     arrays=arrays, launches=launches, data_size=int(data_size), arena_size=int(arena_size), varena_size=int(varena_size),
                     stats=stats, front_of_pos=front_of_pos, border_rows=border_rows)


def execute_numpy(plan: FrontPlan, panels: np.ndarray, rhs: np.ndarray):
    A = plan.arrays
    P = panels.astype(np.float64).copy()
    S = plan.S
    cb: Dict[int, np.ndarray] = {}
    w, b, first, poff = A["f_w"], A["f_b"], A["f_first"], A["f_panel_off"]

    def rel_of(c):
        return A["f_rel"][A["rel_ptr"][c]:A["rel_ptr"][c + 1]]

    def kids(t):
        return A["child_list"][A["child_ptr"][t]:A["child_ptr"][t + 1]]
    for (d, cls, s0, cnt) in plan.launches[:, :4]:
        for t in A["sched"][s0:s0 + cnt]:
            wt, bt = int(w[t]), int(b[t])
            r = wt + bt
            F = np.zeros((r, r))
            F[:, :wt] = P[poff[t]:poff[t] + r * wt].reshape(r, wt)
            for c in kids(t):
                rel = rel_of(c)
                C = np.tril(cb.pop(int(c)))
                F[np.ix_(rel, rel)] += C
            F = np.tril(F)
            L11 = np.linalg.cholesky(F[:wt, :wt] + np.tril(F[:wt, :wt], -1).T)
            F[:wt, :wt] = L11
            if bt:
                L21 = np.linalg.solve(L11, F[wt:, :wt].T).T
                F[wt:, :wt] = L21
                cb[int(t)] = F[wt:, wt:] + np.tril(F[wt:, wt:], -1).T - L21 @ L21.T
            P[poff[t]:poff[t] + r * wt] = F[:, :wt].reshape(-1)
    y = rhs[plan.perm].astype(np.float64).copy()
    ub: Dict[int, np.ndarray] = {}
    for (d, cls, s0, cnt) in plan.launches[:, :4]:
        for t in A["sched"][s0:s0 + cnt]:
            wt, bt = int(w[t]), int(b[t])
            r = wt + bt
            Lp = P[poff[t]:poff[t] + r * wt].reshape(r, wt)
            u = np.zeros(r)
            u[:wt] = y[first[t]:first[t] + wt]
            for c in kids(t):
                u[rel_of(c)] += ub.pop(int(c))
            yt = np.linalg.solve(np.tril(Lp[:wt]), u[:wt])
            y[first[t]:first[t] + wt] = yt
            if bt:
                ub[int(t)] = u[wt:] - Lp[wt:] @ yt
    x = y
    for (d, cls, s0, cnt) in plan.launches[::-1, :4]:
        for t in A["sched"][s0:s0 + cnt]:
            wt, bt = int(w[t]), int(b[t])
            r = wt + bt
            Lp = P[poff[t]:poff[t] + r * wt].reshape(r, wt)
            rows = A["f_rows"][A["rows_ptr"][t]:A["rows_ptr"][t + 1]]
            tt = x[first[t]:first[t] + wt] - (Lp[wt:].T @ x[rows] if bt else 0.0)
            x[first[t]:first[t] + wt] = np.linalg.solve(np.tril(Lp[:wt]).T, tt)
    out = np.empty(plan.n)
    out[plan.perm] = x
    return out, P
```

theseus_b200/sparse_solver.py:

```python
import ctypes as C
import os
from typing import Any, Dict, Optional, Type, Union

import numpy as np
import torch

from . import _lib
from .autograd import LinearSolveFunction, wants_grad
from .core import Objective
from .optimizer import (Linearization, LinearSolver, SparseLinearization, convert_to_alpha_beta_damping_tensors)
from .frontal import build_front_plan
from .sparse import LANE_DIMS, analyze, gram_out_offsets, piece_solve_lists, root_lane_lists, root_split, tile_lane_lists
from .structure import ata_block_structure, build_gram_plan


_ROOT_LAYOUTS = ("lane_root", "lane_tiled_root")
_TILED_LAYOUTS = ("lane_tiled", "lane_tiled_root")


class BaspachoSparseSolver(LinearSolver):
    def __init__(self, objective: Objective, linearization_cls: Optional[Type[Linearization]] = None,
                 linearization_kwargs: Optional[Dict[str, Any]] = None, num_solver_contexts=1, batch_size: Optional[int] = None,
                 auto_reset: bool = True, dev: Optional[str] = None, ordering: str = "mindeg", layout: Optional[str] = None,
                 supernodal_solve: bool = False, front_options: Optional[Dict[str, Any]] = None, **kwargs):
        linearization_cls = linearization_cls or SparseLinearization
        if not linearization_cls == SparseLinearization:
            raise RuntimeError(
                "BaspachoSparseSolver only works with theseus.optimizer.SparseLinearization,"
                + f" got {type(self.linearization)}")
        super().__init__(objective, linearization_cls, linearization_kwargs, **kwargs)
        self.linearization: SparseLinearization = self.linearization
        self._ordering = ordering
        self._layout = layout
        self._supernodal_solve = bool(supernodal_solve)
        self._front_options = dict(front_options or {})
        self._plan = None
        self._dev = None
        self.param_size = None
        self.reset()

    @classmethod
    def from_structure(cls, structure, ordering: str = "mindeg", layout: Optional[str] = None,
                       supernodal_solve: bool = False, front_options: Optional[Dict[str, Any]] = None) -> "BaspachoSparseSolver":
        class _Lin:
            def __init__(self, S):
                self._S, self.A_val, self.b = S, None, None
                self.A_row_ptr, self.A_col_ind = S.A_row_ptr, S.A_col_ind
                self.num_rows, self.num_cols = S.num_rows, S.num_cols

            def structure(self):
                return self._S
        self = cls.__new__(cls)
        self.linearization = _Lin(structure)
        self._ordering, self._plan, self._dev, self._layout = ordering, None, None, layout
        self._supernodal_solve = bool(supernodal_solve)
        self._front_options = dict(front_options or {})
        self.param_size = None
        self.reset()
        return self

    def reset(self, **kwargs):
        if self._plan is not None:
            return
        S = self.linearization.structure()
        if getattr(self, "param_size", None) is None:
            param_size, ptrs, inds = ata_block_structure(S)
            self.param_size, self.block_ptrs, self.block_inds = param_size, ptrs, inds
        param_size, ptrs, inds = self.param_size, self.block_ptrs, self.block_inds
        if self._layout is None:
            return
        if self._layout == "front":
            opts = {k: v for k, v in getattr(self, "_front_options", {}).items() if k != "chunk"}
            for env, key, cast in (("THB_FRONT_TAU", "tau", float), ("THB_FRONT_MERGE_FLOPS", "merge_flops", float),
                                   ("THB_FRONT_MERGE_MAX_R", "merge_max_r", int)):
                if env in os.environ and key not in opts:
                    opts[key] = cast(os.environ[env])
            self._plan = build_front_plan(param_size, ptrs, inds, ordering="auto" if self._ordering == "mindeg" else self._ordering, **opts)
            from .structure import lower_blocks
            blocks, _ = lower_blocks(S, self._plan.pos)
            dims_of = S.var_dims
            f, self._ata_size = self._plan.gram_compact_offsets([(a, b, int(dims_of[a]), int(dims_of[b])) for a, b in blocks])
            self._gram_arrays = build_gram_plan(S, out_offsets=f, pos=self._plan.pos)
            return
        self._plan = analyze(param_size, ptrs, inds, ordering=self._ordering)
        self._gram_arrays = build_gram_plan(S, out_offsets=gram_out_offsets(self._plan), pos=self._plan.pos)

    def layout_for(self, B: int) -> str:
        if self._layout is None:
            self._layout = os.environ.get("THB_SPARSE_LAYOUT") or ("front" if B >= 32 else "item")
            self.reset()
        if self._layout == "front":
            return "front"
        lane_ok = all(int(d) in LANE_DIMS for d in self._plan.dims)
        if self._layout is not None:
            if self._layout not in ("lane", "item", "lane_root", "lane_tiled", "lane_tiled_root"):
                raise ValueError(f"layout must be 'lane', 'item', 'lane_root', 'lane_tiled' or 'lane_tiled_root', got {self._layout}")
            if self._layout != "item" and not lane_ok:
                raise ValueError(f"layout='{self._layout}' needs block sizes in {LANE_DIMS}")
            if self._layout in _ROOT_LAYOUTS and self._root_split() is None:
                raise ValueError(f"layout='{self._layout}': this structure has no dense root (top chain too short)")
            return self._layout
        return "lane" if (lane_ok and B >= 32) else "item"

    def _root_split(self):
        if not hasattr(self, "_root"):
            sp = root_split(self._plan)
            self._root = None if sp is None else (sp,) + root_lane_lists(self._plan, sp)
        return self._root

    @property
    def symbolic_stats(self):
        if self._plan is None:
            self._layout = os.environ.get("THB_SPARSE_LAYOUT") or "front"
            self.reset()
        return dict(self._plan.stats)

    @property
    def effective_layout(self):
        return self._layout

    def _device_plan(self, device):
        if self._dev is not None and self._dev["device"] == device:
            return self._dev
        if self._layout == "front":
            return self._device_plan_front(device)
        P = self._plan
        dev = {k: torch.from_numpy(np.ascontiguousarray(v)).to(device) for k, v in P.arrays.items()}
        st = _lib.SparsePlanStruct(N=P.N, num_levels=int(P.stats["levels"]), max_dim=int(P.dims.max()) if P.N else 0, reserved=0,
                                   n=P.n, data_size=P.data_size, winv_size=P.winv_size,
                                   **{k: dev[k].data_ptr() for k in dev})
        g = self._gram_arrays
        gdev = {k: torch.from_numpy(np.ascontiguousarray(v)).to(device) for k, v in g.items() if isinstance(v, np.ndarray)}
        gst = _lib.make_gram_plan(g, gdev)
        ln = P.lane
        lst, ldev, launches = self._lane_struct(ln, dev, device)
        self._dev = dict(device=device, plan=st, keep=dev, gram=gst, gkeep=gdev, bufs={}, lane=lst, lkeep=(ldev, launches))
        if self._layout in _ROOT_LAYOUTS:
            sp, rl, rr = self._root_split()
            qdev = {k: torch.from_numpy(np.ascontiguousarray(v)).to(device) for k, v in rr.items() if isinstance(v, np.ndarray) and k != "segments"}
            segs = np.ascontiguousarray(rr["segments"], dtype=np.int32)
            qst = _lib.SparseLaneRootStruct(
                num_blocks=int(rr["rb_off"].shape[0]), num_cols=int(rr["root_cols"].shape[0]), nt=int(rr["nt"]), root_start=int(rr["root_start"]),
                num_segments=int(segs.shape[0]), segments=segs.ctypes.data, rb_off=qdev["rb_off"].data_ptr(), rb_row=qdev["rb_row"].data_ptr(),
                rb_col=qdev["rb_col"].data_ptr(), rb_di=qdev["rb_di"].data_ptr(), rb_dj=qdev["rb_dj"].data_ptr(), rf_p0=qdev["rf_p0"].data_ptr(),
                rf_p1=qdev["rf_p1"].data_ptr(), root_cols=qdev["root_cols"].data_ptr(), root_dims=qdev["root_dims"].data_ptr())
            self._dev.update(root=qst, qkeep=(qdev, segs), nt=int(rr["nt"]))
            if self._layout == "lane_root":
                rst, rdev, rlaunch = self._lane_struct(rl, dev, device)
                self._dev.update(lane_root=rst, rkeep=(rdev, rlaunch))
        if self._layout in _TILED_LAYOUTS:
            tl, tt = self._tile_lists()
            tst, tdev, tlaunch = self._lane_struct(tl, dev, device)
            ttdev = {k: torch.from_numpy(np.ascontiguousarray(v)).to(device) for k, v in tt.items()}
            tiles = _lib.SparseLaneTilesStruct(num_tiles=int(tt["tile_tgt"].shape[0]), num_steps=int(tt["step_src"].shape[0]),
                                               tile_tgt=ttdev["tile_tgt"].data_ptr(), step_ptr=ttdev["step_ptr"].data_ptr(),
                                               step_src=ttdev["step_src"].data_ptr())
            self._dev.update({self._layout: tst}, tiles=tiles, tkeep=(tdev, tlaunch, ttdev))
        if getattr(self, "_supernodal_solve", False) and all(int(d) in LANE_DIMS for d in P.dims):
            ps = piece_solve_lists(P, cut=self._root_split()[0]["cut"] if self._layout in _ROOT_LAYOUTS else None)
            pdev = {k: torch.from_numpy(np.ascontiguousarray(ps[k] if k != "width" else ps[k].astype(np.int32))).to(device)
                    for k in ("first", "width", "fr_ext_end", "bc_int_end", "order")}
            plaunch = np.ascontiguousarray(ps["launches"][:, 1:], dtype=np.int32)
            pst = _lib.SparseLanePiecesStruct(num_pieces=int(ps["first"].shape[0]), num_launches=int(plaunch.shape[0]), launches=plaunch.ctypes.data,
                                              **{k: pdev[k].data_ptr() for k in pdev})
            self._dev.update(pieces=pst, pkeep=(pdev, plaunch, ps))
        return self._dev

    def _device_plan_front(self, device):
        P = self._plan
        dev = {k: torch.from_numpy(np.ascontiguousarray(v)).to(device) for k, v in P.arrays.items()}
        st = _lib.FrontPlanStruct(S=P.S, n=P.n, data_size=P.data_size, arena_size=P.arena_size, varena_size=P.varena_size,
                                  **{k: dev[k].data_ptr() for k in ("f_w", "f_b", "f_first", "f_class", "f_wpad", "f_np", "f_cb_ld", "f_depth",
                                                                    "f_panel_off", "f_cb_off", "f_fr_off", "f_u_off", "child_ptr", "child_list",
                                                                    "rel_ptr", "f_rel", "rows_ptr", "f_rows", "sched", "perm", "c_jw", "c_sp_ptr", "c_sp", "c_inv_ptr", "c_inv", "fd", "pc", "pmap")})
        g = self._gram_arrays
        gdev = {k: torch.from_numpy(np.ascontiguousarray(v)).to(device) for k, v in g.items() if isinstance(v, np.ndarray)}
        launches = np.ascontiguousarray(P.launches, dtype=np.int64)
        big = launches[launches[:, 1] == 3]
        self._dev = dict(device=device, front=st, keep=dev, gram=_lib.make_gram_plan(g, gdev), gkeep=gdev, bufs={}, launches=launches,
                         max_np=int(big[:, 5].max()) if len(big) else 0)
        return self._dev

    def _numeric_front(self, A_val, b, alpha, beta, forward=False):
        B, device = A_val.shape[0], A_val.device
        d = self._device_plan(device)
        P = self._plan
        lib = _lib.load()
        s = _lib.stream_ptr()
        chunk = int(min(B, self._front_options.get("chunk", int(os.environ.get("THB_FRONT_CHUNK", "1024")))))
        if d["bufs"].get("key") != (B, "front"):
            ws_bytes = int(lib.thb_potrf_partial_workspace_bytes(chunk, d["max_np"])) if d["max_np"] else 0
            d["bufs"] = dict(key=(B, "front"), chunk=chunk, factor=torch.empty(B, P.data_size, dtype=torch.float64, device=device),
                             ata=torch.empty(B, self._ata_size, dtype=torch.float64, device=device),
                             arena=torch.empty(2, chunk, P.arena_size, dtype=torch.float64, device=device),
                             varena=torch.empty(2, chunk, P.varena_size, dtype=torch.float64, device=device),
                             work=torch.empty(B, P.n, dtype=torch.float64, device=device),
                             ws=torch.empty(max(ws_bytes, 8), dtype=torch.uint8, device=device),
                             Atb=torch.empty(B, P.n, dtype=torch.float64, device=device),
                             AtA_diag=torch.empty(B, P.n, dtype=torch.float64, device=device),
                             info=torch.empty(B, dtype=torch.int32, device=device))
        bufs = d["bufs"]
        factor, Atb, info = bufs["factor"], bufs["Atb"], bufs["info"]
        lin = self.linearization
        if getattr(lin, "_Atb", None) is Atb:
            lin._Atb = lin._AtA_diag = None
        nnz, m = A_val.shape[1], b.shape[1]
        self._factor_stamp = getattr(self, "_factor_stamp", 0) + 1
        ata = bufs["ata"]
        _lib.check(lib.thb_gram_f64(C.byref(d["gram"]), B, _lib.ptr(A_val), nnz, _lib.ptr(b), m, _lib.ptr(ata), self._ata_size,
                                    _lib.ptr(Atb), _lib.ptr(bufs["AtA_diag"]), s), "gram(front)")
        L = d["launches"]
        for c0 in range(0, B, chunk):
            nb = min(chunk, B - c0)
            args = (C.byref(d["front"]), L.ctypes.data, L.shape[0], _lib.ptr(factor[c0:]), _lib.ptr(ata[c0:]), self._ata_size,
                    _lib.ptr(alpha[c0:]) if alpha is not None else None,
                    _lib.ptr(beta[c0:]) if beta is not None else None, _lib.ptr(bufs["arena"]), _lib.ptr(bufs["ws"]) if d["max_np"] else None,
                    bufs["ws"].numel(), _lib.ptr(info[c0:]))
            if forward:
                _lib.check(lib.thb_front_factor_forward_f64(*args, _lib.ptr(Atb[c0:]), _lib.ptr(bufs["work"][c0:]), _lib.ptr(bufs["varena"]), nb, s),
                           "front_factor_forward")
            else:
                _lib.check(lib.thb_front_factor_f64(*args, nb, s), "front_factor")
        self._keep = (A_val, b, alpha, beta)
        return Atb

    def _substitute_front(self, rhs):
        d, P = self._dev, self._plan
        bufs = d["bufs"]
        B, chunk = bufs["key"][0], bufs["chunk"]
        lib = _lib.load()
        rhs = rhs.contiguous()
        x = torch.empty(B, P.n, dtype=torch.float64, device=rhs.device)
        L = d["launches"]
        for c0 in range(0, B, chunk):
            nb = min(chunk, B - c0)
            _lib.check(lib.thb_front_solve_f64(C.byref(d["front"]), L.ctypes.data, L.shape[0], _lib.ptr(bufs["factor"][c0:]), _lib.ptr(rhs[c0:]),
                                               _lib.ptr(x[c0:]), _lib.ptr(bufs["work"][c0:]), _lib.ptr(bufs["varena"]), nb, _lib.stream_ptr()),
                       "front_solve")
        return x

    def _backward_front(self):
        d, P = self._dev, self._plan
        bufs = d["bufs"]
        B, chunk = bufs["key"][0], bufs["chunk"]
        lib = _lib.load()
        x = torch.empty(B, P.n, dtype=torch.float64, device=bufs["work"].device)
        L = d["launches"]
        for c0 in range(0, B, chunk):
            nb = min(chunk, B - c0)
            _lib.check(lib.thb_front_backward_f64(C.byref(d["front"]), L.ctypes.data, L.shape[0], _lib.ptr(bufs["factor"][c0:]), _lib.ptr(x[c0:]),
                                                  _lib.ptr(bufs["work"][c0:]), nb, _lib.stream_ptr()), "front_backward")
        return x

    def _lane_struct(self, ln, dev, device):
        P = self._plan
        ldev = {k: torch.from_numpy(np.ascontiguousarray(v)).to(device) for k, v in ln.items() if k != "launches"}
        launches = np.ascontiguousarray(ln["launches"], dtype=np.int32)
        lst = _lib.SparseLanePlanStruct(
            N=P.N, n=P.n, data_size=P.data_size, diag_size=P.winv_size, num_launches=int(launches.shape[0]),
            launches=launches.ctypes.data, dims=dev["dims"].data_ptr(), col_start=dev["col_start"].data_ptr(),
            pstart=dev["pstart"].data_ptr(), dl_off=dev["winv_off"].data_ptr(), diag_off=dev["diag_off"].data_ptr(),
            up_a=dev["up_a"].data_ptr(), up_b=dev["up_b"].data_ptr(), up_k=dev["up_k"].data_ptr(),
            u_tgt=ldev["u_tgt"].data_ptr(), u_p0=ldev["u_p0"].data_ptr(), u_p1=ldev["u_p1"].data_ptr(),
            t_off=ldev["t_off"].data_ptr(), t_diag=ldev["t_diag"].data_ptr(), t_dl=ldev["t_dl"].data_ptr(),
            t_pstart=ldev["t_pstart"].data_ptr(), s_col=ldev["s_col"].data_ptr(),
            fr_ptr=dev["fr_ptr"].data_ptr(), fr_off=dev["fr_off"].data_ptr(), fr_p=ldev["fr_p"].data_ptr(), fr_d=ldev["fr_d"].data_ptr(),
            bc_ptr=dev["bc_ptr"].data_ptr(), bc_off=dev["bc_off"].data_ptr(), bc_p=ldev["bc_p"].data_ptr(), bc_d=ldev["bc_d"].data_ptr())
        return lst, ldev, launches

    def _tile_lists(self):
        if not hasattr(self, "_tiles"):
            self._tiles = tile_lane_lists(self._plan, self._root_split()[0] if self._layout in _ROOT_LAYOUTS else None)
        return self._tiles

    def solve(self, damping: Optional[Union[float, torch.Tensor]] = None, ellipsoidal_damping: bool = True,
              damping_eps: float = 1e-8, **kwargs) -> torch.Tensor:
        lin = self.linearization
        A_val, b = lin.A_val, lin.b
        if A_val is None:
            raise RuntimeError("linearize() must be called before solve()")
        if wants_grad(A_val, b):
            detach = bool(getattr(lin, "detached_hessian", False))
            return LinearSolveFunction.apply(A_val, b, self, damping, ellipsoidal_damping, damping_eps, detach)
        x = self._solve_nograd(A_val, b, damping, ellipsoidal_damping, damping_eps)[0]
        bufs = self._dev["bufs"] if self._dev is not None else {}
        if "AtA_diag" in bufs and A_val.dtype == torch.float64 and A_val.is_contiguous() and b.is_contiguous() and getattr(lin, "_Atb", 0) is None:
            lin._Atb, lin._AtA_diag = bufs["Atb"], bufs["AtA_diag"]
        return x

    def _solve_nograd(self, A_val, b, damping, ellipsoidal_damping, damping_eps):
        out_dtype = A_val.dtype
        A64, b64 = A_val.detach(), b.detach()
        if A64.dtype != torch.float64:
            A64, b64 = A64.double(), b64.double()
        A64, b64 = A64.contiguous(), b64.contiguous()
        alpha = beta = None
        if damping is not None:
            alpha, beta = convert_to_alpha_beta_damping_tensors(damping, damping_eps, ellipsoidal_damping, A64.shape[0], A64.device, torch.float64)
        if self.layout_for(A64.shape[0]) == "front":
            self._numeric_front(A64, b64, alpha, beta, forward=True)
            x = self._backward_front()
        else:
            Atb = self._numeric(A64, b64, alpha, beta)
            x = self._substitute(Atb)
        self._last_info = self._dev["bufs"]["info"]
        if not getattr(self, "defer_info_check", False):
            self.check_info()
        return x.to(out_dtype), (A64, b64, x, alpha, beta)

    def check_info(self, x=None):
        self._raise_if_bad(self._last_info)
        return x

    @staticmethod
    def _raise_if_bad(info):
        bad = info.nonzero()
        if bad.numel() > 0:
            k = int(bad[0, 0])
            raise RuntimeError(f"block-sparse Cholesky: batch element {k}: matrix is not positive definite (pivot {int(info[k])})")

    def _numeric(self, A_val, b, alpha, beta):
        B, device = A_val.shape[0], A_val.device
        layout = self.layout_for(B)
        if layout == "front":
            return self._numeric_front(A_val, b, alpha, beta)
        d = self._device_plan(device)
        P = self._plan
        lib = _lib.load()
        s = _lib.stream_ptr()
        key = (B, layout)
        if d["bufs"].get("key") != key:
            Bp = int(lib.thb_sparse_lane_padded_batch(B))
            shape = (lambda k: (k, Bp)) if layout != "item" else (lambda k: (B, k))
            d["bufs"] = dict(key=key, factor=torch.empty(shape(P.data_size), dtype=torch.float64, device=device),
                             diag=torch.empty(shape(P.winv_size), dtype=torch.float64, device=device),
                             work=torch.empty(shape(P.n), dtype=torch.float64, device=device),
                             Atb=torch.empty(B, P.n, dtype=torch.float64, device=device),
                             info=torch.empty(B, dtype=torch.int32, device=device))
            if layout in _ROOT_LAYOUTS:
                nt = d["nt"]
                d["bufs"].update(S=torch.empty(B, nt, nt, dtype=torch.float64, device=device),
                                 ws=torch.empty(int(lib.thb_potrf_workspace_bytes(B, nt)), dtype=torch.uint8, device=device),
                                 rhs_root=torch.empty(B, nt, dtype=torch.float64, device=device),
                                 x_root=torch.empty(B, nt, dtype=torch.float64, device=device),
                                 info_root=torch.empty(B, dtype=torch.int32, device=device))
        bufs = d["bufs"]
        factor, diag, Atb, info = bufs["factor"], bufs["diag"], bufs["Atb"], bufs["info"]
        nnz, m = A_val.shape[1], b.shape[1]
        self._factor_stamp = getattr(self, "_factor_stamp", 0) + 1
        _lib.check(lib.thb_fill_zero(_lib.ptr(factor), factor.numel() * 8, s), "fill_zero")
        if layout != "item":
            lplan = d[layout]
            _lib.check(lib.thb_sparse_lane_gram_f64(C.byref(d["gram"]), B, _lib.ptr(A_val), nnz, _lib.ptr(factor), s), "gram(lane)")
            _lib.check(lib.thb_gram_f64(C.byref(d["gram"]), B, _lib.ptr(A_val), nnz, _lib.ptr(b), m, None, 0, _lib.ptr(Atb), None, s), "Atb")
            if alpha is not None:
                _lib.check(lib.thb_sparse_lane_damp_f64(C.byref(d["lane"]), _lib.ptr(factor), _lib.ptr(alpha), _lib.ptr(beta), B, s), "lane_damp")
            if layout in _TILED_LAYOUTS:
                _lib.check(lib.thb_sparse_lane_factor_tiled_f64(C.byref(lplan), C.byref(d["tiles"]), _lib.ptr(factor), _lib.ptr(diag), _lib.ptr(info),
                                                                B, s), "lane_factor_tiled")
            else:
                _lib.check(lib.thb_sparse_lane_factor_f64(C.byref(lplan), _lib.ptr(factor), _lib.ptr(diag), _lib.ptr(info), B, s), "lane_factor")
            if layout in _ROOT_LAYOUTS:
                _lib.check(lib.thb_sparse_lane_root_gather_f64(C.byref(d["root"]), _lib.ptr(factor), _lib.ptr(bufs["S"]), B, s), "root_gather")
                _lib.check(lib.thb_potrf_f64(_lib.ptr(bufs["S"]), None, None, _lib.ptr(bufs["info_root"]), B, d["nt"], _lib.ptr(bufs["ws"]),
                                             bufs["ws"].numel(), s), "root_potrf")
                torch.maximum(info, torch.where(bufs["info_root"] > 0, bufs["info_root"] + int(self._root[2]["root_start"]), bufs["info_root"]),
                              out=info)
        else:
            _lib.check(lib.thb_gram_f64(C.byref(d["gram"]), B, _lib.ptr(A_val), nnz, _lib.ptr(b), m, _lib.ptr(factor), P.data_size,
                                        _lib.ptr(Atb), None, s), "gram(sparse)")
            if alpha is not None:
                _lib.check(lib.thb_sparse_damp_f64(C.byref(d["plan"]), _lib.ptr(factor), _lib.ptr(alpha), _lib.ptr(beta), B, s), "sparse_damp")
            _lib.check(lib.thb_sparse_factor_f64(C.byref(d["plan"]), _lib.ptr(factor), _lib.ptr(diag), _lib.ptr(info), B, s), "sparse_factor")
        self._keep = (A_val, b, alpha, beta)
        return Atb

    def _substitute(self, rhs: torch.Tensor) -> torch.Tensor:
        d, P = self._dev, self._plan
        bufs = d["bufs"]
        B, layout = bufs["key"]
        if layout == "front":
            return self._substitute_front(rhs)
        lib = _lib.load()
        rhs = rhs.contiguous()
        x = torch.empty(B, P.n, dtype=torch.float64, device=rhs.device)
        pieces = C.byref(d["pieces"]) if (layout != "item" and "pieces" in d) else None
        if layout in ("lane", "lane_tiled") and pieces is not None:
            s = _lib.stream_ptr()
            lp, F, D, W = C.byref(d[layout]), _lib.ptr(bufs["factor"]), _lib.ptr(bufs["diag"]), _lib.ptr(bufs["work"])
            _lib.check(lib.thb_sparse_lane_piece_forward_f64(lp, pieces, F, D, _lib.ptr(rhs), W, B, s), "piece_forward")
            _lib.check(lib.thb_sparse_lane_piece_backward_f64(lp, pieces, F, D, W, _lib.ptr(x), B, s), "piece_backward")
        elif layout in ("lane", "lane_tiled"):
            _lib.check(lib.thb_sparse_lane_solve_f64(C.byref(d[layout]), _lib.ptr(bufs["factor"]), _lib.ptr(bufs["diag"]), _lib.ptr(rhs), _lib.ptr(x),
                                                     _lib.ptr(bufs["work"]), B, _lib.stream_ptr()), "lane_solve")
        elif layout in _ROOT_LAYOUTS:
            s = _lib.stream_ptr()
            lp, rt = C.byref(d[layout]), C.byref(d["root"])
            F, D, W = _lib.ptr(bufs["factor"]), _lib.ptr(bufs["diag"]), _lib.ptr(bufs["work"])
            if pieces is not None:
                _lib.check(lib.thb_sparse_lane_piece_forward_f64(lp, pieces, F, D, _lib.ptr(rhs), W, B, s), "piece_forward")
            else:
                _lib.check(lib.thb_sparse_lane_forward_f64(lp, F, D, _lib.ptr(rhs), W, B, s), "lane_forward")
            _lib.check(lib.thb_sparse_lane_root_rhs_f64(lp, rt, F, _lib.ptr(rhs), W, _lib.ptr(bufs["rhs_root"]), B, s), "root_rhs")
            _lib.check(lib.thb_potrs_f64(_lib.ptr(bufs["rhs_root"]), _lib.ptr(bufs["x_root"]), B, d["nt"], _lib.ptr(bufs["ws"]), bufs["ws"].numel(), s),
                       "root_potrs")
            _lib.check(lib.thb_sparse_lane_root_scatter_f64(lp, rt, _lib.ptr(bufs["x_root"]), W, _lib.ptr(x), B, s), "root_scatter")
            if pieces is not None:
                _lib.check(lib.thb_sparse_lane_piece_backward_f64(lp, pieces, F, D, W, _lib.ptr(x), B, s), "piece_backward")
            else:
                _lib.check(lib.thb_sparse_lane_backward_f64(lp, F, D, W, _lib.ptr(x), B, s), "lane_backward")
        else:
            _lib.check(lib.thb_sparse_solve_f64(C.byref(d["plan"]), _lib.ptr(bufs["factor"]), _lib.ptr(bufs["diag"]), _lib.ptr(rhs), _lib.ptr(x),
                                                _lib.ptr(bufs["work"]), B, _lib.stream_ptr()), "sparse_solve")
        return x


BlockSparseSolver = BaspachoSparseSolver
CholmodSparseSolver = BaspachoSparseSolver
LUCudaSparseSolver = BaspachoSparseSolver
```

Before: 4.969.

## Fuse chains of small supernodal fronts into a single chain kernel launch

Adds a front_chain_kernel that factors a chain of small fronts (parent-child pieces) inside one thread block, applying earlier pieces' updates directly from global factor data instead of writing and reading contribution blocks through the arena between launches. A separate factor plan with chain headers and factor_launches is built and used for the numeric factorization and forward paths. The goal is fewer per-depth kernel launches and less arena traffic in the multifrontal Cholesky, at the cost of redundant global reads of prior panels and lower parallelism within each chain.

Result: no change. 4.957 (median of 6 runs) (-0.2%).

```diff
diff --git a/theseus_b200/_lib.py b/theseus_b200/_lib.py
--- a/theseus_b200/_lib.py
+++ b/theseus_b200/_lib.py
@@ -82,6 +82,11 @@
     _fields_ = [("S", c_i64), ("n", c_i64), ("data_size", c_i64), ("arena_size", c_i64), ("varena_size", c_i64)] + [(k, c_vp) for k in (
         "f_w", "f_b", "f_first", "f_class", "f_wpad", "f_np", "f_cb_ld", "f_depth", "f_panel_off", "f_cb_off", "f_fr_off", "f_u_off",
         "child_ptr", "child_list", "rel_ptr", "f_rel", "rows_ptr", "f_rows", "sched", "perm", "c_jw", "c_sp_ptr", "c_sp", "c_inv_ptr", "c_inv", "fd", "pc", "pmap")]
+
+
+def make_front_plan(P, dev) -> FrontPlanStruct:
+    return FrontPlanStruct(S=P.S, n=P.n, data_size=P.data_size, arena_size=P.arena_size, varena_size=P.varena_size,
+                           **{k: dev[k].data_ptr() for k, _ in FrontPlanStruct._fields_[5:]})
 
 
 _PF = C.POINTER(FrontPlanStruct)
diff --git a/theseus_b200/csrc/thb_front.cu b/theseus_b200/csrc/thb_front.cu
--- a/theseus_b200/csrc/thb_front.cu
+++ b/theseus_b200/csrc/thb_front.cu
@@ -238,6 +238,204 @@
       u[i * us] -= s;
     }
     __syncthreads();
+  }
+}
+
+
+template <int THREADS>
+__device__ __forceinline__ void front_load_children(const FrontArgs& a, const int64_t* PC0, int nch, int r, int64_t item, FrontChild* ch,
+                                                    int32_t* INV, double* sm, int fill, int tid) {
+  const thb_front_plan& p = a.p;
+  for (int q = 0; q < nch; q++) {
+    const int64_t* PC = PC0 + (int64_t)q * 6;
+    const double* csrc = a.arena_child + item * p.arena_size + PC[0];
+    const int cld = (int)(PC[1] & 0xffffffffLL);
+    if (tid == 0) {
+      ch[q].src = csrc;
+      ch[q].ldg = cld;
+      ch[q].lo = (int)PC[2];
+      ch[q].hi = (int)PC[3];
+      ch[q].uoff = (int)PC[5];
+    }
+    const int32_t* inv = p.c_inv + PC[4];
+    for (int l = tid; l < r; l += THREADS) INV[q * r + l] = inv[l];
+  }
+  for (int e = tid; e < fill; e += THREADS) sm[e] = 0.0;
+}
+
+template <int THREADS>
+__device__ __forceinline__ void front_assemble(const FrontArgs& a, double* PN, int ldp, int w, int w8, int r, const double* Lg, int64_t f_panel_off,
+                                               int64_t item, const FrontChild* ch, const int32_t* INV, int nch, int tid) {
+  if (tid < w8 - w) PN[(w + tid) * ldp + w + tid] = 1.0;
+  const double al = a.alpha != nullptr ? a.alpha[item] : 0.0;
+  const double be = a.beta != nullptr ? a.beta[item] : 0.0;
+  const int total = r * w;
+  for (int e0 = tid; e0 < total; e0 += FRONT_PL * THREADS) {
+    int ii[FRONT_PL], jj[FRONT_PL];
+    double v[FRONT_PL];
+#pragma unroll
+    for (int u = 0; u < FRONT_PL; u++) {
+      const int e = e0 + u * THREADS;
+      ii[u] = e / w;
+      jj[u] = e - ii[u] * w;
+      if (e >= total || jj[u] > ii[u]) ii[u] = -1;
+      v[u] = ii[u] >= 0 ? front_panel_in(a, Lg, f_panel_off, item, e) : 0.0;
+    }
+#pragma unroll
+    for (int u = 0; u < FRONT_PL; u++)
+      if (ii[u] >= 0 && ii[u] == jj[u]) v[u] = v[u] + (al * v[u] + be);
+    for (int q = 0; q < nch; q++) {
+      const double* src = ch[q].src;
+      const int ldg = ch[q].ldg, lo = ch[q].lo, hi = ch[q].hi;
+      const int32_t* inv = INV + q * r;
+#pragma unroll
+      for (int u = 0; u < FRONT_PL; u++) {
+        if (ii[u] >= lo && jj[u] <= hi) {
+          const int ci = inv[ii[u]], cj = inv[jj[u]];
+          if (ci >= 0 && cj >= 0) v[u] += src[(int64_t)ci * ldg + cj];
+        }
+      }
+    }
+#pragma unroll
+    for (int u = 0; u < FRONT_PL; u++)
+      if (ii[u] >= 0) PN[(ii[u] < w ? ii[u] : ii[u] + (w8 - w)) * ldp + jj[u]] = v[u];
+  }
+}
+
+template <int THREADS>
+__device__ __forceinline__ void front_gather_u(const FrontArgs& a, double* U, int ldp, int w, int r, int f_first, int64_t item, const FrontChild* ch,
+                                               const int32_t* INV, int nch, const double* prev, int tid) {
+  const thb_front_plan& p = a.p;
+  for (int i = tid; i < r; i += THREADS) {
+    double v = i < w ? a.rhs[item * p.n + p.perm[f_first + i]] : 0.0;
+    for (int q = 0; q < nch; q++) {
+      if (i >= ch[q].lo && i <= ch[q].hi) {
+        const int k = INV[q * r + i];
+        if (k >= 0) v += a.v_child[item * p.varena_size + ch[q].uoff + k];
+      }
+    }
+    if (prev != nullptr) v += prev[i];
+    U[i * ldp] = v;
+  }
+}
+
+template <int THREADS>
+__device__ __forceinline__ void front_factor_panel(double* PN, int ldp, int w, int w8, int b16, double* Wd, int f_first, int32_t* info, int warp,
+                                                   int lane) {
+  constexpr int NW = THREADS / 32;
+  const int nbk = w8 / 8, nrt = (w8 + b16) / 8;
+  for (int jb = 0; jb < nbk; jb++) {
+    if (warp == 0) front_diag_block(PN, ldp, jb, Wd, lane, w, f_first, info);
+    __syncthreads();
+    const int npair = (nrt - jb) / 2;
+    for (int q = warp; q < npair; q += NW) front_tile_column<true>(PN, ldp, jb, jb + 1 + 2 * q, Wd, lane);
+    __syncthreads();
+  }
+}
+
+template <int THREADS>
+__device__ __forceinline__ void front_write_panel(double* Lg, const double* PN, int ldp, int w, int w8, int r, int tid) {
+  int i = tid / w, j = tid - i * w;
+  const int di = THREADS / w, dj = THREADS - di * w;
+  for (int e = tid; e < r * w; e += THREADS) {
+    Lg[e] = (j > i) ? 0.0 : PN[(i < w ? i : i + (w8 - w)) * ldp + j];
+    i += di; j += dj;
+    if (j >= w) { j -= w; i++; }
+  }
+}
+
+__device__ __forceinline__ void front_acc_global(double (&acc)[2][2][2], const double* L, int wj, int rj, int ra, int rb, int lane) {
+  const int lr = lane >> 2, lc = lane & 3;
+  const bool va0 = ra + lr < rj, va1 = ra + 8 + lr < rj, vb0 = rb + lr < rj, vb1 = rb + 8 + lr < rj;
+  const double* Pa = L + (int64_t)(ra + lr) * wj + lc;
+  const double* Pb = L + (int64_t)(rb + lr) * wj + lc;
+  const int64_t s8 = 8 * (int64_t)wj;
+#pragma unroll 4
+  for (int k4 = 0; k4 < wj; k4 += 4) {
+    const bool km = k4 + lc < wj;
+    const double a0 = (va0 && km) ? Pa[k4] : 0.0, a1 = (va1 && km) ? Pa[s8 + k4] : 0.0;
+    const double b0 = (vb0 && km) ? Pb[k4] : 0.0, b1 = (vb1 && km) ? Pb[s8 + k4] : 0.0;
+    front_mma884(acc[0][0][0], acc[0][0][1], a0, b0);
+    front_mma884(acc[0][1][0], acc[0][1][1], a0, b1);
+    front_mma884(acc[1][0][0], acc[1][0][1], a1, b0);
+    front_mma884(acc[1][1][0], acc[1][1][1], a1, b1);
+  }
+}
+
+template <int THREADS>
+__device__ __forceinline__ void front_update_tiles(double* dst, int ldg_out, const double* PN, int ldp, int w, int w8, int b, int r, const FrontChild* ch,
+                                                   const int32_t* INV, int nch, const int64_t* PRE, int npre, const double* fac, int f_first,
+                                                   int warp, int lane) {
+  constexpr int NW = THREADS / 32;
+  const int lr = lane >> 2, lc = lane & 3;
+  const int b16 = (b + 15) & ~15;
+  const double* P = PN + w8 * ldp;
+  const int nmt = b16 / 16, ntl = nmt * (nmt + 1) / 2;
+  for (int q = warp; q < ntl; q += NW) {
+    int R = (int)((sqrtf(8.0f * (float)q + 1.0f) - 1.0f) * 0.5f);
+    while ((R + 1) * (R + 2) / 2 <= q) R++;
+    while (R * (R + 1) / 2 > q) R--;
+    const int ct = q - R * (R + 1) / 2;
+    double gch[2][2][2] = {{{0.0, 0.0}, {0.0, 0.0}}, {{0.0, 0.0}, {0.0, 0.0}}};
+    const int li0 = w + 16 * R + lr, lj0 = w + 16 * ct + 2 * lc;
+    for (int qc = 0; qc < nch; qc++) {
+      if (w + 16 * R + 15 >= ch[qc].lo && w + 16 * ct <= ch[qc].hi) {
+        const int32_t* inv = INV + qc * r;
+        const double* src = ch[qc].src;
+        const int ldg = ch[qc].ldg;
+        int ci[2], cj[2][2];
+#pragma unroll
+        for (int mi = 0; mi < 2; mi++) ci[mi] = (li0 + 8 * mi < r) ? inv[li0 + 8 * mi] : -1;
+#pragma unroll
+        for (int ni = 0; ni < 2; ni++)
+#pragma unroll
+          for (int u = 0; u < 2; u++) cj[ni][u] = (lj0 + 8 * ni + u < r) ? inv[lj0 + 8 * ni + u] : -1;
+#pragma unroll
+        for (int mi = 0; mi < 2; mi++)
+#pragma unroll
+          for (int ni = 0; ni < 2; ni++)
+#pragma unroll
+            for (int u = 0; u < 2; u++)
+              if (ci[mi] >= 0 && cj[ni][u] >= 0 && cj[ni][u] <= ci[mi]) gch[mi][ni][u] += src[(int64_t)ci[mi] * ldg + cj[ni][u]];
+      }
+    }
+    double acc[2][2][2] = {{{0.0, 0.0}, {0.0, 0.0}}, {{0.0, 0.0}, {0.0, 0.0}}};
+    const double* Pa = P + (16 * R + lr) * ldp + lc;
+    const double* Pb = P + (16 * ct + lr) * ldp + lc;
+    for (int k4 = 0; k4 < w8; k4 += 4) {
+      const double a0 = Pa[k4], a1 = Pa[8 * ldp + k4];
+      const double b0 = Pb[k4], b1 = Pb[8 * ldp + k4];
+      front_mma884(acc[0][0][0], acc[0][0][1], a0, b0);
+      front_mma884(acc[0][1][0], acc[0][1][1], a0, b1);
+      front_mma884(acc[1][0][0], acc[1][0][1], a1, b0);
+      front_mma884(acc[1][1][0], acc[1][1][1], a1, b1);
+    }
+    for (int j = 0; j < npre; j++) {
+      const int64_t* F = PRE + (int64_t)j * 8;
+      const int wj = (int)F[1], off = f_first - (int)F[3] + w;
+      front_acc_global(acc, fac + F[4], wj, wj + (int)F[2], off + 16 * R, off + 16 * ct, lane);
+    }
+#pragma unroll
+    for (int mi = 0; mi < 2; mi++)
+#pragma unroll
+      for (int ni = 0; ni < 2; ni++) {
+        acc[mi][ni][0] = gch[mi][ni][0] - acc[mi][ni][0];
+        acc[mi][ni][1] = gch[mi][ni][1] - acc[mi][ni][1];
+      }
+#pragma unroll
+    for (int mi = 0; mi < 2; mi++) {
+      const int i = 16 * R + 8 * mi + lr;
+      if (i < b) {
+        double* drow = dst + (int64_t)i * ldg_out;
+#pragma unroll
+        for (int ni = 0; ni < 2; ni++)
+#pragma unroll
+          for (int u = 0; u < 2; u++) {
+            const int jj = 16 * ct + 8 * ni + 2 * lc + u;
+            if (jj <= i) drow[jj] = acc[mi][ni][u];
+          }
+      }
+    }
   }
 }
 
@@ -444,6 +642,81 @@
   }
 }
 
+template <int THREADS>
+__global__ void __launch_bounds__(THREADS, 1) front_chain_kernel(FrontArgs a) {
+  extern __shared__ double sm[];
+  const thb_front_plan& p = a.p;
+  const int tid = threadIdx.x, lane = tid & 31, warp = tid >> 5;
+  constexpr int NW = THREADS / 32;
+  const int lr = lane >> 2, lc = lane & 3;
+  const int64_t item = blockIdx.x;
+  THB_PDL_TRIGGER();
+  const int64_t* H = p.fd + (int64_t)(a.s0 + blockIdx.y) * 8;
+  const int npc = (int)H[0];
+  const int64_t* PR = p.fd + H[1] * 8;
+  double* fac = a.factor + item * p.data_size;
+  double* ub = a.rhs != nullptr ? a.v_cur + item * p.varena_size + H[5] : nullptr;
+  THB_PDL_WAIT();
+  for (int k = 0; k < npc; k++) {
+    const int64_t* FD = PR + (int64_t)k * 8;
+    const int w = (int)FD[1], b = (int)FD[2], r = w + b;
+    const int f_first = (int)FD[3];
+    const int64_t f_panel_off = FD[4];
+    const int nch = min((int)FD[6], FRONT_MAX_CHILDREN), n_own = (int)FD[7];
+    const int b16 = (b + 15) & ~15, w8 = (w + 7) & ~7;
+    const int ldp = front_pad_ld(w8);
+    const int prow = w8 + b16 + 8;
+    double* PN = sm;
+    double* Wd = PN + prow * ldp;
+    FrontChild* ch = reinterpret_cast<FrontChild*>(Wd + 8 * FRONT_WD_LD);
+    int32_t* INV = reinterpret_cast<int32_t*>(Wd + 8 * FRONT_WD_LD + 3 * FRONT_MAX_CHILDREN);
+    __syncthreads();
+    front_load_children<THREADS>(a, p.pc + FD[5] * 6, nch, r, item, ch, INV, sm, prow * ldp, tid);
+    __syncthreads();
+    double* Lg = fac + f_panel_off;
+    front_assemble<THREADS>(a, PN, ldp, w, w8, r, Lg, f_panel_off, item, ch, INV, nch, tid);
+    double* U = PN + w8;
+    if (a.rhs != nullptr) front_gather_u<THREADS>(a, U, ldp, w, r, f_first, item, ch, INV, n_own, k > 0 ? ub : nullptr, tid);
+    __syncthreads();
+    const int nrt = (r + 15) / 16, nct = (w + 15) / 16;
+    for (int q = warp; k > 0 && q < nrt * nct; q += NW) {
+      const int R = q / nct, ct = q - R * nct;
+      if (R < ct) continue;
+      double acc[2][2][2] = {{{0.0, 0.0}, {0.0, 0.0}}, {{0.0, 0.0}, {0.0, 0.0}}};
+      for (int j = 0; j < k; j++) {
+        const int64_t* F = PR + (int64_t)j * 8;
+        const int wj = (int)F[1], off = f_first - (int)F[3];
+        front_acc_global(acc, fac + F[4], wj, wj + (int)F[2], off + 16 * R, off + 16 * ct, lane);
+      }
+#pragma unroll
+      for (int mi = 0; mi < 2; mi++) {
+        const int i = 16 * R + 8 * mi + lr;
+        if (i < r) {
+          double* row = PN + (i < w ? i : i + (w8 - w)) * ldp;
+#pragma unroll
+          for (int ni = 0; ni < 2; ni++)
+#pragma unroll
+            for (int u = 0; u < 2; u++) {
+              const int c = 16 * ct + 8 * ni + 2 * lc + u;
+              if (c < w && c <= i) row[c] -= acc[mi][ni][u];
+            }
+        }
+      }
+    }
+    __syncthreads();
+    front_factor_panel<THREADS>(PN, ldp, w, w8, b16, Wd, f_first, a.info + item, warp, lane);
+    front_write_panel<THREADS>(Lg, PN, ldp, w, w8, r, tid);
+    if (a.rhs != nullptr) {
+      front_forward_elim<THREADS>(FrontRowsPanel{PN, ldp, w, w8 - w}, U, ldp, w, r, tid, lane);
+      for (int i = tid; i < w; i += THREADS) a.work[item * p.n + f_first + i] = U[i * ldp];
+      for (int i = tid; i < b; i += THREADS) ub[i] = U[(w + i) * ldp];
+    }
+    if (k == npc - 1 && b > 0)
+      front_update_tiles<THREADS>(a.arena_cur + item * p.arena_size + H[3], (int)H[4], PN, ldp, w, w8, b, r, ch, INV, nch, PR, k, fac, f_first,
+                                  warp, lane);
+  }
+}
+
 constexpr int ASM_ROWS = 16, ASM_THREADS = 256;
 
 __device__ __forceinline__ int front_map_big(int l, int w, int wpad) { return l < w ? l : wpad + (l - w); }
@@ -776,7 +1049,7 @@
   if (B > 65535LL * 32768LL) return THB_ERR_UNSUPPORTED;
   cudaStream_t cs = thb_cs(stream);
   THB_CUDA(cudaMemsetAsync(info, 0, (size_t)B * 4, cs));
-  static size_t smem_set[5] = {0, 0, 0, 0, 0}, asm_set = 0;
+  static size_t smem_set[5] = {0, 0, 0, 0, 0}, chain_set[2] = {0, 0}, asm_set = 0;
   static const int thr_cls[2] = {[] { const char* e = getenv("THB_FRONT_T0"); const int v = e ? atoi(e) : 64; return (v == 128 || v == 256) ? v : 64; }(),
                                  [] { const char* e = getenv("THB_FRONT_T1"); const int v = e ? atoi(e) : 128; return v == 256 ? 256 : 128; }()};
   static int front_prefetch_flag = -1;
@@ -797,7 +1070,22 @@
     a.rhs = rhs; a.work = work;
     a.v_cur = rhs != nullptr ? varena + (int64_t)(depth & 1) * B * p->varena_size : nullptr;
     a.v_child = rhs != nullptr ? varena + (int64_t)((depth + 1) & 1) * B * p->varena_size : nullptr;
-    if (cls < 3) {
+    if (cls == 4) {
+      const size_t smem = (size_t)L[4];
+#ifndef THB_SIMT_EMU
+      if (smem > 227 * 1024) return THB_ERR_UNSUPPORTED;
+#endif
+      if (count > 65535) return THB_ERR_UNSUPPORTED;
+      const dim3 grid((unsigned)B, (unsigned)count);
+      if (smem <= 56 * 1024) {
+        int rc = front_set_smem(front_chain_kernel<256>, smem, &chain_set[0]); if (rc) return rc;
+        FRONT_LAUNCH(front_chain_kernel<256>, grid, 256, smem, cs, a);
+      } else {
+        int rc = front_set_smem(front_chain_kernel<512>, smem, &chain_set[1]); if (rc) return rc;
+        FRONT_LAUNCH(front_chain_kernel<512>, grid, 512, smem, cs, a);
+      }
+      THB_CHECK_LAUNCH();
+    } else if (cls < 3) {
       const size_t smem = (size_t)L[4];
 #ifndef THB_SIMT_EMU
       if (smem > 227 * 1024) return THB_ERR_UNSUPPORTED;
diff --git a/theseus_b200/extlib.py b/theseus_b200/extlib.py
--- a/theseus_b200/extlib.py
+++ b/theseus_b200/extlib.py
@@ -41,13 +41,13 @@
         if self._dev is None:
             P = self.plan
             dev = {k: torch.from_numpy(np.ascontiguousarray(v)).to(self.device) for k, v in P.arrays.items()}
-            keys = ("f_w", "f_b", "f_first", "f_class", "f_wpad", "f_np", "f_cb_ld", "f_depth", "f_panel_off", "f_cb_off", "f_fr_off", "f_u_off",
-                    "child_ptr", "child_list", "rel_ptr", "f_rel", "rows_ptr", "f_rows", "sched", "perm", "c_jw", "c_sp_ptr", "c_sp", "c_inv_ptr", "c_inv", "fd", "pc", "pmap")
-            st = _lib.FrontPlanStruct(S=P.S, n=P.n, data_size=P.data_size, arena_size=P.arena_size, varena_size=P.varena_size,
-                                      **{k: dev[k].data_ptr() for k in keys})
+            st = _lib.make_front_plan(P, dev)
+            fdev = {k: torch.from_numpy(np.ascontiguousarray(v)).to(self.device) if v is not P.arrays[k] else dev[k] for k, v in P.factor_arrays.items()}
             launches = np.ascontiguousarray(P.launches, dtype=np.int64)
             big = launches[launches[:, 1] == 3]
-            self._dev = dict(front=st, keep=dev, launches=launches, max_np=int(big[:, 5].max()) if len(big) else 0)
+            self._dev = dict(front=st, keep=dev, launches=launches, max_np=int(big[:, 5].max()) if len(big) else 0,
+                             front_factor=_lib.make_front_plan(P, fdev), fkeep=fdev,
+                             factor_launches=np.ascontiguousarray(P.factor_launches, dtype=np.int64))
         return self._dev
 
     def _offset_of(self, r: np.ndarray, c: np.ndarray) -> np.ndarray:
@@ -152,8 +152,8 @@
 
     def factor(self):
         dev, bufs, lib = self.sym._device_plan(), self._buffers(), _lib.load()
-        L = dev["launches"]
-        _lib.check(lib.thb_front_factor_f64(C.byref(dev["front"]), L.ctypes.data, L.shape[0], _lib.ptr(self.data), None, 0, None, None, _lib.ptr(bufs["arena"]),
+        L = dev["factor_launches"]
+        _lib.check(lib.thb_front_factor_f64(C.byref(dev["front_factor"]), L.ctypes.data, L.shape[0], _lib.ptr(self.data), None, 0, None, None, _lib.ptr(bufs["arena"]),
                                             _lib.ptr(bufs["ws"]) if dev["max_np"] else None, bufs["ws"].numel(), _lib.ptr(bufs["info"]), self.B,
                                             _lib.stream_ptr()), "front_factor")
         bad = bufs["info"].nonzero()
diff --git a/theseus_b200/frontal.py b/theseus_b200/frontal.py
--- a/theseus_b200/frontal.py
+++ b/theseus_b200/frontal.py
@@ -177,6 +177,9 @@
     stats: Dict[str, float] = field(default_factory=dict)
     front_of_pos: np.ndarray = None
     border_rows: List[np.ndarray] = None
+    factor_launches: np.ndarray = None
+    factor_arrays: Dict[str, np.ndarray] = None
+    chains: List[dict] = None
 
     def gram_compact_offsets(self, blocks_dims):
         f = self.gram_out_offsets()
@@ -282,6 +285,7 @@
                     break
     fr_cols: List[List[int]] = []
     fr_below: List[np.ndarray] = []
+    chain_ranges: List[tuple] = []
     for sidx in (q for q in range(S0) if alive[q]):
         cs, bl = cols[sidx], np.asarray(below[sidx], dtype=np.int64)
         wtot, btot = int(dims0[cs].sum()), (int(dims0[bl].sum()) if len(bl) else 0)
@@ -303,9 +307,12 @@
         if any(small_smem_bytes(int(dims0[cs[a:b_]].sum()), int(dims0[cs[b_:]].sum()) + btot, 4) > SMALL_SMEM_LIMIT for a, b_ in pieces):
             fr_cols.append(list(cs)); fr_below.append(bl)
             continue
+        t0 = len(fr_cols)
         for a, b_ in pieces:
             fr_cols.append(list(cs[a:b_]))
             fr_below.append(np.concatenate([np.asarray(cs[b_:], dtype=np.int64), bl]))
+        if len(pieces) > 1:
+            chain_ranges.append((t0, len(fr_cols)))
     S = len(fr_cols)
     keep = list(range(S))
     cols, below = fr_cols, fr_below
@@ -490,19 +497,170 @@
             pc[int(child_ptr[t]) + k] = (int(f_cb_off[c]), int(f_cb_ld[c]) | (int(f_b[c]) << 32), int(rel[0]), int(rel[-1]), int(c_inv_ptr[c]),
                                          int(f_u_off[c]))
     flops = float(sum(_front_cost(float(f_w[t]), float(f_b[t])) for t in range(S)))
-    stats = dict(ordering=oname, column_flops=col_flops, flops=flops, nnz_L=float(sum(int(f_r[t]) * int(f_w[t]) for t in range(S))),
-                 fronts=float(S), max_front=float(f_r.max()) if S else 0.0, depth=float(max_depth + 1), big_fronts=float((f_class == 3).sum()),
-                 launches=float(len(launches)), cb_doubles=float(sum(int(b) * int(b) for b in f_b)), levels=float(max_depth + 1),
-                 num_updates=0.0, num_chains=float(S), chain_levels=float(max_depth + 1))
     arrays = dict(f_w=f_w, f_b=f_b, f_first=f_first, f_parent=f_parent, f_depth=f_depth, f_class=f_class, f_panel_off=f_panel_off,
                   f_wpad=f_wpad, f_np=f_np, f_cb_off=f_cb_off, f_cb_ld=f_cb_ld, f_fr_off=f_fr_off, f_u_off=f_u_off,
                   child_ptr=child_ptr, child_list=np.array(child_list, dtype=np.int32), rel_ptr=rel_ptr, f_rel=f_rel,
                   rows_ptr=rows_ptr, f_rows=f_rows, sched=sched, perm=perm.astype(np.int32), c_jw=c_jw, c_sp_ptr=c_sp_ptr, c_sp=c_sp,
                   c_inv_ptr=c_inv_ptr, c_inv=c_inv, fd=fd.reshape(-1), pc=pc.reshape(-1),
                   pmap=-np.ones(max(int(data_size), 1), dtype=np.int32))
+    chains = _chain_records(chain_ranges, arrays, children) if CHAIN_FACTOR else []
+    if chains:
+        fx = _factor_schedule(chains, arrays, children, f_bucket)
+        factor_launches, farena, fvarena = fx.pop("launches"), fx.pop("arena_size"), fx.pop("varena_size")
+        arena_size, varena_size = max(arena_size, farena), max(varena_size, fvarena)
+        factor_arrays = dict(arrays, **fx)
+        fdepth = int(factor_launches[:, 0].max()) + 1
+        cb_doubles = sum(int(f_b[t]) ** 2 for t in range(S)) - sum(int(f_b[t]) ** 2 for c in chains if c["chain_path"] for t in c["pieces"][:-1])
+    else:
+        factor_launches, factor_arrays, fdepth, cb_doubles = launches, arrays, max_depth + 1, sum(int(b) * int(b) for b in f_b)
+    stats = dict(ordering=oname, column_flops=col_flops, flops=flops, nnz_L=float(sum(int(f_r[t]) * int(f_w[t]) for t in range(S))),
+                 fronts=float(S), max_front=float(f_r.max()) if S else 0.0, depth=float(fdepth), big_fronts=float((f_class == 3).sum()),
+                 launches=float(len(factor_launches)), cb_doubles=float(cb_doubles), levels=float(max_depth + 1),
+                 num_updates=0.0, num_chains=float(S), chain_levels=float(max_depth + 1),
+                 split_chains=float(len(chains)), chain_path=float(sum(1 for c in chains if c["chain_path"])))
     return FrontPlan(N=N, n=n, param_size=param_size, order=order, pos=pos, dims=dims, pstart=pstart, col_start=col_start, perm=perm, S=S,
                      arrays=arrays, launches=launches, data_size=int(data_size), arena_size=int(arena_size), varena_size=int(varena_size),
-                     stats=stats, front_of_pos=front_of_pos, border_rows=border_rows)
+                     stats=stats, front_of_pos=front_of_pos, border_rows=border_rows, factor_launches=factor_launches,
+                     factor_arrays=factor_arrays, chains=chains)
+
+
+CHAIN_FACTOR = __import__("os").environ.get("THB_FRONT_CHAIN", "0") == "1"
+CHAIN_KIND = 4
+
+
+def _chain_records(chain_ranges, A, children):
+    w, b, first = A["f_w"], A["f_b"], A["f_first"]
+    out = []
+    for t0, t1 in chain_ranges:
+        pieces = list(range(t0, t1))
+        real = {t: [c for c in children[t] if not (t > t0 and c == t - 1)] for t in pieces}
+        phases, smem = [], 0
+        for k, t in enumerate(pieces):
+            lst = [(c, 0) for c in real[t]]
+            n_own = len(lst)
+            for tj in pieces[:k]:
+                off = int(first[t] - first[tj])
+                hi_col = off + int(w[t]) if t != pieces[-1] else 1 << 40
+                for c in real[tj]:
+                    rel = A["f_rel"][A["rel_ptr"][c]:A["rel_ptr"][c + 1]]
+                    if np.any((rel >= off) & (rel < hi_col)):
+                        lst.append((int(c), off))
+            phases.append((lst, n_own))
+            smem = max(smem, small_smem_bytes(int(w[t]), int(b[t]), len(lst)))
+        ok = all(len(l) <= SMALL_MAX_CHILDREN for l, _ in phases) and smem <= SMALL_SMEM_LIMIT and \
+            all(int(A["f_class"][t]) < 3 for t in pieces)
+        out.append(dict(pieces=pieces, phases=phases, smem=int(smem), chain_path=bool(ok)))
+    return out
+
+
+def _factor_schedule(chains, A, children, f_bucket):
+    S = int(A["f_w"].shape[0])
+    w, b, first, par, cls = A["f_w"], A["f_b"], A["f_first"], A["f_parent"], A["f_class"]
+    r = w + b
+    unit_of = np.arange(S)
+    units = [[t] for t in range(S)]
+    for ci, c in enumerate(chains):
+        if c["chain_path"]:
+            for t in c["pieces"]:
+                unit_of[t] = c["pieces"][-1]
+            units[c["pieces"][-1]] = list(c["pieces"])
+            for t in c["pieces"][:-1]:
+                units[t] = None
+    chain_of_last = {c["pieces"][-1]: c for c in chains if c["chain_path"]}
+    depth = np.zeros(S, dtype=np.int64)
+    for u in range(S - 1, -1, -1):
+        if units[u] is not None and par[u] >= 0:
+            depth[u] = depth[unit_of[par[u]]] + 1
+    live = [u for u in range(S) if units[u] is not None]
+    max_depth = int(max(depth[u] for u in live))
+    f_wpad, f_np = A["f_wpad"], A["f_np"]
+    f_cb_off = np.zeros(S, dtype=np.int64)
+    f_cb_ld = np.zeros(S, dtype=np.int32)
+    f_fr_off = np.zeros(S, dtype=np.int64)
+    f_u_off = np.zeros(S, dtype=np.int64)
+    arena, varena = [0, 0], [0, 0]
+    for d in range(max_depth, -1, -1):
+        a = v = 0
+        for u in (q for q in live if depth[q] == d):
+            if cls[u] == 3:
+                wp, npad = int(f_wpad[u]), int(f_np[u])
+                f_fr_off[u] = a
+                f_cb_off[u] = a + wp * npad + wp
+                f_cb_ld[u] = npad
+                a += npad * npad
+            else:
+                ld = int(b[u]) + (int(b[u]) & 1)
+                f_cb_off[u] = a
+                f_cb_ld[u] = ld
+                a += int(b[u]) * ld
+            bv = int(b[units[u][0]])
+            f_u_off[units[u]] = v
+            v += bv + (bv & 1)
+        arena[d & 1] = max(arena[d & 1], a)
+        varena[d & 1] = max(varena[d & 1], v)
+    child_ptr = A["child_ptr"]
+    pc = A["pc"].reshape(-1, 6).copy()
+    for t in range(S):
+        for k, c in enumerate(children[t]):
+            q = int(child_ptr[t]) + k
+            pc[q, 0], pc[q, 1], pc[q, 5] = f_cb_off[c], int(f_cb_ld[c]) | (int(b[c]) << 32), f_u_off[c]
+    singles = sorted((u for u in live if u not in chain_of_last), key=lambda t: (-int(depth[t]), int(cls[t]), int(f_bucket[t]), -int(r[t]), t))
+    fd_rows, pc_rows, launches = [], [], []
+    hdr, pieces_fd = [], []
+    npc = pc.shape[0]
+    by_depth = {}
+    for u in singles:
+        by_depth.setdefault(int(depth[u]), []).append(u)
+    chains_at = {}
+    for u, c in chain_of_last.items():
+        chains_at.setdefault(int(depth[u]), []).append(c)
+    n_single = len(singles)
+    sched = np.array(singles, dtype=np.int32)
+    pos_of = {u: i for i, u in enumerate(singles)}
+    chain_rows = []
+    for d in range(max_depth, -1, -1):
+        cs = sorted(chains_at.get(d, []), key=lambda c: -int(r[c["pieces"][0]]))
+        if cs:
+            launches.append((d, CHAIN_KIND, n_single + len(hdr), len(cs), max(c["smem"] for c in cs), max(int(r[c["pieces"][0]]) for c in cs),
+                             0, 0, 0, 0, 0, 0))
+            for c in cs:
+                hdr.append(c)
+        grp = by_depth.get(d, [])
+        i = 0
+        while i < len(grp):
+            t = grp[i]
+            j = i + 1
+            if cls[t] != 3:
+                while j < len(grp) and int(cls[grp[j]]) == int(cls[t]) and int(f_bucket[grp[j]]) == int(f_bucket[t]):
+                    j += 1
+                qs = grp[i:j]
+                smem = max(small_smem_bytes(int(w[q]), int(b[q]), len(children[q])) for q in qs)
+                launches.append((d, int(cls[t]), pos_of[t], j - i, smem, max(int(r[q]) for q in qs), max(int(r[q]) * int(w[q]) for q in qs),
+                                 0, 0, 0, 0, 0))
+            else:
+                launches.append((d, 3, pos_of[t], 1, 0, int(f_np[t]), int(f_wpad[t]) // BIG_TW, int(f_fr_off[t]), int(first[t]), t, int(w[t]),
+                                 int(b[t])))
+            i = j
+    fd = np.zeros((n_single + len(hdr) + sum(len(c["pieces"]) for c in hdr), 8), dtype=np.int64)
+    for q, t in enumerate(singles):
+        cb, ce = int(child_ptr[t]), int(child_ptr[t + 1])
+        fd[q] = (t, int(w[t]), int(b[t]), int(first[t]), int(A["f_panel_off"][t]), int(f_cb_off[t]), int(f_cb_ld[t]), cb | ((ce - cb) << 32))
+    prow = n_single + len(hdr)
+    extra = []
+    for h, c in enumerate(hdr):
+        last = c["pieces"][-1]
+        fd[n_single + h] = (len(c["pieces"]), prow, int(b[last]), int(f_cb_off[last]), int(f_cb_ld[last]), int(f_u_off[last]), c["smem"], 0)
+        for t, (lst, n_own) in zip(c["pieces"], c["phases"]):
+            fd[prow] = (t, int(w[t]), int(b[t]), int(first[t]), int(A["f_panel_off"][t]), npc + len(extra), len(lst), n_own)
+            prow += 1
+            for (ch, off) in lst:
+                rel = A["f_rel"][A["rel_ptr"][ch]:A["rel_ptr"][ch + 1]]
+                extra.append((int(f_cb_off[ch]), int(f_cb_ld[ch]) | (int(b[ch]) << 32), max(int(rel[0]) - off, 0), int(rel[-1]) - off,
+                              int(A["c_inv_ptr"][ch]) + off, int(f_u_off[ch])))
+    if extra:
+        pc = np.concatenate([pc, np.array(extra, dtype=np.int64)])
+    return dict(f_cb_off=f_cb_off, f_cb_ld=f_cb_ld, f_fr_off=f_fr_off, f_u_off=f_u_off, fd=fd.reshape(-1), pc=pc.reshape(-1), sched=sched,
+                launches=np.array(launches, dtype=np.int64).reshape(-1, 12), arena_size=int(max(arena) + 2), varena_size=int(max(varena) + 2))
 
 
 def execute_numpy(plan: FrontPlan, panels: np.ndarray, rhs: np.ndarray):
@@ -562,3 +720,70 @@
     out = np.empty(plan.n)
     out[plan.perm] = x
     return out, P
+
+
+def factor_numpy(plan: FrontPlan, panels: np.ndarray):
+    A = plan.factor_arrays
+    P = panels.astype(np.float64).copy()
+    w, b, poff, c_inv = A["f_w"], A["f_b"], A["f_panel_off"], A["c_inv"]
+    fd, pc = A["fd"].reshape(-1, 8), A["pc"].reshape(-1, 6)
+    arena = np.full((2, plan.arena_size), np.nan)
+
+    def gather(F, d, recs, r):
+        for rec in recs:
+            inv = c_inv[rec[4]:rec[4] + r]
+            ld, bc = int(rec[1] & 0xffffffff), int(rec[1] >> 32)
+            C = arena[(d + 1) & 1, rec[0]:rec[0] + bc * ld].reshape(bc, ld)[:, :bc]
+            rows = np.nonzero(inv >= 0)[0]
+            ci = inv[rows]
+            blk = C[np.ix_(ci, ci)]
+            F[np.ix_(rows, rows)] += np.where(ci[None, :] <= ci[:, None], blk, 0.0)
+
+    def put_cb(d, off, ld, C):
+        bc = C.shape[0]
+        arena[d & 1, off:off + bc * ld].reshape(bc, ld)[:, :bc] = np.tril(C)
+
+    for (d, kind, s0, cnt) in plan.factor_launches[:, :4]:
+        for q in range(s0, s0 + cnt):
+            if kind != CHAIN_KIND:
+                t, wt, bt = int(fd[q, 0]), int(fd[q, 1]), int(fd[q, 2])
+                r = wt + bt
+                F = np.zeros((r, r))
+                F[:, :wt] = P[poff[t]:poff[t] + r * wt].reshape(r, wt)
+                F[:wt, :wt] = np.tril(F[:wt, :wt])
+                cb, ce = int(fd[q, 7] & 0xffffffff), int(fd[q, 7] >> 32)
+                gather(F, d, pc[cb:cb + ce], r)
+                F = np.tril(F)
+                L11 = np.linalg.cholesky(F[:wt, :wt] + np.tril(F[:wt, :wt], -1).T)
+                F[:wt, :wt] = L11
+                if bt:
+                    L21 = np.linalg.solve(L11, F[wt:, :wt].T).T
+                    F[wt:, :wt] = L21
+                    put_cb(d, int(fd[q, 5]), int(fd[q, 6]), F[wt:, wt:] - np.tril(L21 @ L21.T))
+                P[poff[t]:poff[t] + r * wt] = F[:, :wt].reshape(-1)
+                continue
+            npc, prow, bf, cb_off, cb_ld = (int(x) for x in fd[q, :5])
+            done = []
+            for k in range(npc):
+                t, wt, bt, ft, po, l0, ln = (int(x) for x in fd[prow + k, :7])
+                r = wt + bt
+                F = np.zeros((r, r))
+                F[:, :wt] = P[po:po + r * wt].reshape(r, wt)
+                F[:wt, :wt] = np.tril(F[:wt, :wt])
+                gather(F, d, pc[l0:l0 + ln], r)
+                for (fj, wj, rj, Lj) in done:
+                    o = ft - fj
+                    F[:, :wt] -= Lj[o:o + r] @ Lj[o:o + wt].T
+                F = np.tril(F)
+                L11 = np.linalg.cholesky(F[:wt, :wt] + np.tril(F[:wt, :wt], -1).T)
+                F[:wt, :wt] = L11
+                F[wt:, :wt] = np.linalg.solve(L11, F[wt:, :wt].T).T
+                P[po:po + r * wt] = F[:, :wt].reshape(-1)
+                done.append((ft, wt, r, F[:, :wt].copy()))
+                if k == npc - 1 and bf:
+                    C = F[wt:, wt:]
+                    for (fj, wj, rj, Lj) in done:
+                        o = ft - fj + wt
+                        C = C - Lj[o:o + bf] @ Lj[o:o + bf].T
+                    put_cb(d, cb_off, cb_ld, C)
+    return P
diff --git a/theseus_b200/sparse_solver.py b/theseus_b200/sparse_solver.py
--- a/theseus_b200/sparse_solver.py
+++ b/theseus_b200/sparse_solver.py
@@ -169,16 +169,15 @@
     def _device_plan_front(self, device):
         P = self._plan
         dev = {k: torch.from_numpy(np.ascontiguousarray(v)).to(device) for k, v in P.arrays.items()}
-        st = _lib.FrontPlanStruct(S=P.S, n=P.n, data_size=P.data_size, arena_size=P.arena_size, varena_size=P.varena_size,
-                                  **{k: dev[k].data_ptr() for k in ("f_w", "f_b", "f_first", "f_class", "f_wpad", "f_np", "f_cb_ld", "f_depth",
-                                                                    "f_panel_off", "f_cb_off", "f_fr_off", "f_u_off", "child_ptr", "child_list",
-                                                                    "rel_ptr", "f_rel", "rows_ptr", "f_rows", "sched", "perm", "c_jw", "c_sp_ptr", "c_sp", "c_inv_ptr", "c_inv", "fd", "pc", "pmap")})
+        st = _lib.make_front_plan(P, dev)
+        fdev = {k: torch.from_numpy(np.ascontiguousarray(v)).to(device) if v is not P.arrays[k] else dev[k] for k, v in P.factor_arrays.items()}
         g = self._gram_arrays
         gdev = {k: torch.from_numpy(np.ascontiguousarray(v)).to(device) for k, v in g.items() if isinstance(v, np.ndarray)}
         launches = np.ascontiguousarray(P.launches, dtype=np.int64)
         big = launches[launches[:, 1] == 3]
         self._dev = dict(device=device, front=st, keep=dev, gram=_lib.make_gram_plan(g, gdev), gkeep=gdev, bufs={}, launches=launches,
-                         max_np=int(big[:, 5].max()) if len(big) else 0)
+                         max_np=int(big[:, 5].max()) if len(big) else 0, front_factor=_lib.make_front_plan(P, fdev), fkeep=fdev,
+                         factor_launches=np.ascontiguousarray(P.factor_launches, dtype=np.int64))
         return self._dev
 
     def _numeric_front(self, A_val, b, alpha, beta, forward=False):
@@ -209,10 +208,10 @@
         ata = bufs["ata"]
         _lib.check(lib.thb_gram_f64(C.byref(d["gram"]), B, _lib.ptr(A_val), nnz, _lib.ptr(b), m, _lib.ptr(ata), self._ata_size,
                                     _lib.ptr(Atb), _lib.ptr(bufs["AtA_diag"]), s), "gram(front)")
-        L = d["launches"]
+        L = d["factor_launches"]
         for c0 in range(0, B, chunk):
             nb = min(chunk, B - c0)
-            args = (C.byref(d["front"]), L.ctypes.data, L.shape[0], _lib.ptr(factor[c0:]), _lib.ptr(ata[c0:]), self._ata_size,
+            args = (C.byref(d["front_factor"]), L.ctypes.data, L.shape[0], _lib.ptr(factor[c0:]), _lib.ptr(ata[c0:]), self._ata_size,
                     _lib.ptr(alpha[c0:]) if alpha is not None else None,
                     _lib.ptr(beta[c0:]) if beta is not None else None, _lib.ptr(bufs["arena"]), _lib.ptr(bufs["ws"]) if d["max_np"] else None,
                     bufs["ws"].numel(), _lib.ptr(info[c0:]))
```
